# chenruduan/OAReactDiff

Measured on AMD Instinct MI355X. Metric: denoising_steps_per_sec, higher is better.
Workload: dtype f32; 1 GPU; EGNNDynamics.forward (LEFTNet H=196 R=96 L=6), B=64 reactions/GPU x 3 objects x 23 atoms, complete graph per reaction (N=4416, E=300288), T=1000 sampler step shape; batch_per_gpu=64, atoms_per_object=23, parallelism=replica x1 (no collective), launch=eager

## Files before the change

### oareactdiff_amd/_capi.py

```python
from __future__ import annotations

import ctypes as C
import os

from .build import LIB

OARD_MAX_OBJECTS = 8
ABI_VERSION = 2040
OARD_OK, OARD_EINVAL, OARD_ENOTCOMPLETE, OARD_EHIP, OARD_ENOMEM = 0, -1, -2, -3, -4
ERRORS = {OARD_EINVAL: "invalid argument / unsupported configuration", OARD_ENOTCOMPLETE: "topology is not complete-per-sample",
          OARD_EHIP: "HIP runtime error", OARD_ENOMEM: "workspace too small"}

PREC_GCL_BF16X3, PREC_EQUI_BF16X3, PREC_TRAIN_BF16X3 = 1, 2, 4
TAP_S, TAP_VEC, TAP_EDGE, TAP_POS_FRAME, TAP_DPOS, TAP_HOUT, TAP_LABELS, TAP_NE1 = 1, 2, 3, 4, 5, 6, 7, 8

EXPORTS = ["oard_version", "oard_supported", "oard_param_count", "oard_packed_bytes", "oard_pack_weights",
           "oard_topology_create", "oard_topology_destroy", "oard_topology_num_nodes", "oard_topology_num_edges",
           "oard_topology_num_inner_edges", "oard_topology_num_samples", "oard_topology_check_edge_index",
           "oard_workspace_bytes", "oard_forward", "oard_active_inner_edges", "oard_debug_lin3u_table", "oard_sampler_step", "oard_sampler_step_dev", "oard_tap", "oard_debug_stop_after", "oard_debug_option", "oard_timing_enable", "oard_timing_reset",
           "oard_timing_get",
           "oard_topology_create_parts", "oard_topology_export", "oard_tape_bytes", "oard_tape_entry", "oard_forward_train",
           "oard_packed_bwd_bytes", "oard_pack_weights_bwd", "oard_gcl_backward_dx", "oard_edge_node_sums",
           "oard_equi_backward_dx", "oard_scalarize_backward", "oard_equi_msg_backward", "oard_lin3u_forward", "oard_lin3u_backward", "oard_wgrad_scratch_bytes", "oard_wgrad",
           "oard_train_scratch_bytes", "oard_train_scratch_poison", "oard_train_scratch_entry", "oard_train_tail_backward",
# ... 46 lines not shown
        raise OardError(f"{LIB} not found: build it with `python -m oareactdiff_amd.build` "
                        "(there is no CPU fallback for the HIP backend)")
    L = C.CDLL(LIB)
    vp, i32, i64, sz = C.c_void_p, C.c_int32, C.c_int64, C.c_size_t
    cfgp = C.POINTER(OardConfig)
    L.oard_version.restype = C.c_int
    got = L.oard_version()
    if got != ABI_VERSION:
        raise OardError(f"{LIB} has ABI version {got}, this package expects {ABI_VERSION}: rebuild it "
                        "(`python -m oareactdiff_amd.build --force`, or the script that made the OARD_LIB build)")
    L.oard_supported.argtypes = [cfgp]; L.oard_supported.restype = C.c_int
    L.oard_param_count.argtypes = [cfgp]; L.oard_param_count.restype = sz
    L.oard_packed_bytes.argtypes = [cfgp]; L.oard_packed_bytes.restype = sz
    L.oard_pack_weights.argtypes = [cfgp, C.POINTER(vp), sz, vp, sz, vp]; L.oard_pack_weights.restype = C.c_int
    L.oard_topology_create.argtypes = [cfgp, C.POINTER(i64), C.POINTER(i64), i64, C.POINTER(vp)]
    L.oard_topology_create.restype = C.c_int
    L.oard_topology_destroy.argtypes = [vp]; L.oard_topology_destroy.restype = None
    for f in ("oard_topology_num_nodes", "oard_topology_num_edges", "oard_topology_num_inner_edges",
              "oard_topology_num_samples"):
        getattr(L, f).argtypes = [vp]; getattr(L, f).restype = i64
    L.oard_topology_check_edge_index.argtypes = [vp, vp, i64, vp, vp]; L.oard_topology_check_edge_index.restype = C.c_int
    L.oard_workspace_bytes.argtypes = [cfgp, vp]; L.oard_workspace_bytes.restype = sz
    L.oard_forward.argtypes = [cfgp, vp, vp, C.POINTER(vp), vp, C.c_int, vp, C.POINTER(vp), vp, sz, vp, vp]
    L.oard_forward.restype = C.c_int
    L.oard_debug_lin3u_table.argtypes = [cfgp, vp, C.c_int, vp, vp]; L.oard_debug_lin3u_table.restype = C.c_int
    L.oard_active_inner_edges.argtypes = [cfgp, vp, vp, sz, C.POINTER(i64), vp]; L.oard_active_inner_edges.restype = C.c_int
    L.oard_sampler_step.argtypes = [cfgp, vp, C.c_int, C.POINTER(vp), C.POINTER(vp), C.POINTER(vp), C.POINTER(vp),
                                    C.c_float, C.c_float, C.c_float, C.c_int, C.POINTER(vp), vp]
    L.oard_sampler_step.restype = C.c_int
    L.oard_sampler_step_dev.argtypes = [cfgp, vp, C.c_int, C.POINTER(vp), C.POINTER(vp), C.POINTER(vp), C.POINTER(vp), vp, C.c_int,
                                        C.POINTER(vp), vp]
    L.oard_sampler_step_dev.restype = C.c_int
    L.oard_tap.argtypes = [cfgp, vp, vp, C.c_int, C.c_int, vp, vp]; L.oard_tap.restype = C.c_int
    ci = C.c_int
    L.oard_topology_create_parts.argtypes = [cfgp, C.POINTER(i64), C.POINTER(i64), i64, ci, C.POINTER(vp)]
    L.oard_topology_create_parts.restype = ci
    L.oard_topology_export.argtypes = [vp, ci, vp, i64, vp]; L.oard_topology_export.restype = ci
    L.oard_tape_bytes.argtypes = [cfgp, vp]; L.oard_tape_bytes.restype = sz
    L.oard_tape_entry.argtypes = [cfgp, vp, ci, ci, C.POINTER(sz), C.POINTER(i64), C.POINTER(i64)]; L.oard_tape_entry.restype = ci
    L.oard_forward_train.argtypes = [cfgp, vp, vp, C.POINTER(vp), vp, ci, vp, C.POINTER(vp), vp, sz, vp, sz, vp, vp]
    L.oard_forward_train.restype = ci
    L.oard_packed_bwd_bytes.argtypes = [cfgp]; L.oard_packed_bwd_bytes.restype = sz
    L.oard_pack_weights_bwd.argtypes = [cfgp, C.POINTER(vp), sz, vp, sz, vp]; L.oard_pack_weights_bwd.restype = ci
    L.oard_gcl_backward_dx.argtypes = [cfgp, vp, vp, ci, vp, vp, vp, vp, vp, vp, vp, vp, vp]; L.oard_gcl_backward_dx.restype = ci
    L.oard_edge_node_sums.argtypes = [cfgp, vp, vp, vp, vp, vp]; L.oard_edge_node_sums.restype = ci
    L.oard_equi_backward_dx.argtypes = [cfgp, vp, vp, ci, vp, vp, vp, vp, vp]; L.oard_equi_backward_dx.restype = ci
    L.oard_scalarize_backward.argtypes = [cfgp, vp, vp, vp, vp, ci, vp, vp, vp, vp]; L.oard_scalarize_backward.restype = ci
    L.oard_equi_msg_backward.argtypes = [cfgp, vp, vp, ci, vp, vp, vp, vp, vp, vp, vp, vp, vp]; L.oard_equi_msg_backward.restype = ci
    L.oard_lin3u_forward.argtypes = [cfgp, vp, ci, vp, i64, vp, vp]; L.oard_lin3u_forward.restype = ci
    L.oard_lin3u_backward.argtypes = [cfgp, vp, ci, vp, vp, i64, vp, vp, vp, vp, vp, vp, vp]; L.oard_lin3u_backward.restype = ci
    L.oard_wgrad_scratch_bytes.argtypes = [ci, ci, i64]; L.oard_wgrad_scratch_bytes.restype = sz
    L.oard_wgrad.argtypes = [vp, ci, ci, ci, ci, ci, vp, ci, ci, ci, ci, ci, ci, i64, vp, vp, vp, sz, vp]; L.oard_wgrad.restype = ci
    pvp = C.POINTER(vp)
    L.oard_train_scratch_bytes.argtypes = [cfgp, vp]; L.oard_train_scratch_bytes.restype = sz
    L.oard_train_scratch_poison.argtypes = [cfgp, vp, vp, sz, vp]; L.oard_train_scratch_poison.restype = ci
    L.oard_train_scratch_entry.argtypes = [cfgp, vp, ci, C.POINTER(sz), C.POINTER(i64), C.POINTER(i64)]; L.oard_train_scratch_entry.restype = ci
    L.oard_train_tail_backward.argtypes = [cfgp, vp, vp, vp, vp, pvp, vp, vp, pvp, pvp, vp, sz, vp]; L.oard_train_tail_backward.restype = ci
    L.oard_train_layer_backward.argtypes = [cfgp, vp, vp, vp, vp, ci, vp, vp, vp, pvp, pvp, vp, sz, vp]; L.oard_train_layer_backward.restype = ci
    L.oard_train_init_backward.argtypes = [cfgp, vp, vp, vp, vp, pvp, vp, vp, pvp, pvp, vp, sz, vp]; L.oard_train_init_backward.restype = ci
    L.oard_train_stage_backward.argtypes = [cfgp, vp, vp, vp, vp, ci, ci, vp, vp, vp, vp, vp, vp, pvp, pvp, vp, sz, vp]
    L.oard_train_stage_backward.restype = ci
    L.oard_nan_replace.argtypes = [cfgp, vp, vp, pvp, pvp, vp]; L.oard_nan_replace.restype = ci
    pf, cf = C.POINTER(C.c_float), C.c_float
    L.oard_loss_prepare.argtypes = [cfgp, vp, pvp, pvp, pvp, pvp, vp, vp, ci, pf, pf, ci, ci, pvp, pvp, vp]; L.oard_loss_prepare.restype = ci
    L.oard_loss_terms.argtypes = [cfgp, vp, pvp, pvp, pvp, pvp, pvp, vp, vp, ci, pf, pf, pf, ci, ci, vp, vp, pvp, vp]; L.oard_loss_terms.restype = ci
    cd = C.c_double
    L.oard_adamw_step.argtypes = [vp, vp, vp, vp, vp, i64, cd, cd, cd, cd, cd, i64, ci, cd, vp]; L.oard_adamw_step.restype = ci
    L.oard_adamw_step_dev.argtypes = [vp, vp, vp, vp, vp, i64, cd, cd, cd, cd, cd, ci, ci, vp, ci, vp, vp, vp, vp]; L.oard_adamw_step_dev.restype = ci
    L.oard_library_stream.argtypes = [ci, pvp]; L.oard_library_stream.restype = ci
    L.oard_graph_create.argtypes = [cfgp, vp, vp, i64, vp, i64, pvp]; L.oard_graph_create.restype = ci
    L.oard_graph_destroy.argtypes = [vp]; L.oard_graph_destroy.restype = None
    L.oard_graph_num_nodes.argtypes = [vp]; L.oard_graph_num_nodes.restype = i64
    L.oard_graph_num_edges.argtypes = [vp]; L.oard_graph_num_edges.restype = i64
    L.oard_graph_object_rows.argtypes = [vp, ci]; L.oard_graph_object_rows.restype = i64
    L.oard_graph_is_complete.argtypes = [vp]; L.oard_graph_is_complete.restype = ci
    L.oard_graph_workspace_bytes.argtypes = [cfgp, vp]; L.oard_graph_workspace_bytes.restype = sz
    L.oard_graph_forward.argtypes = [cfgp, vp, pvp, sz, pvp, vp, ci, vp, pvp, vp, sz, vp, vp]; L.oard_graph_forward.restype = ci
    L.oard_debug_stop_after.argtypes = [C.c_int]; L.oard_debug_stop_after.restype = C.c_int
    L.oard_debug_option.argtypes = [C.c_char_p, C.c_int]; L.oard_debug_option.restype = C.c_int
    L.oard_timing_enable.argtypes = [C.c_int]; L.oard_timing_enable.restype = C.c_int
    L.oard_timing_reset.argtypes = []; L.oard_timing_reset.restype = C.c_int
    L.oard_timing_get.argtypes = [C.c_char_p, C.POINTER(C.c_double), C.POINTER(i64)]; L.oard_timing_get.restype = C.c_int
    for env, opt in (("OARD_GCL_VARIANT", b"gcl_variant"), ("OARD_EQUI_VARIANT", b"equi_variant"),
                     ("OARD_NODE_VARIANT", b"node_variant"), ("OARD_GCL_SKIP", b"gcl_skip"), ("OARD_EQUI_SKIP", b"equi_skip"), ("OARD_EQUI_L0_SKIP", b"equi_l0_skip"), ("OARD_GCL_PERSIST", b"gcl_persist"), ("OARD_GCL_GRID", b"gcl_grid"), ("OARD_PARTS", b"parts"), ("OARD_SEQUENTIAL", b"sequential"), ("OARD_POISON", b"poison"), ("OARD_AUTO_SMALL", b"auto_small"), ("OARD_AUTO_TINY", b"auto_tiny"), ("OARD_NPB", b"npb"),
                     ("OARD_WGRAD_WGS", b"wgrad_wgs"), ("OARD_WGRAD_LDS", b"wgrad_lds"), ("OARD_WGRAD_T16", b"wgrad_t16"), ("OARD_WGRAD_QUEUE", b"wgrad_queue"), ("OARD_GATE_FOLD", b"gate_fold"), ("OARD_WGRAD_SHAPES", b"wgrad_shapes"), ("OARD_TRAIN_DUAL", b"train_dual"), ("OARD_SMALL_SPLIT", b"small_split"),
                     ("OARD_SKIP_FAMILIES", b"skip_families")):
        if os.environ.get(env) not in (None, ""):
            check(L.oard_debug_option(opt, int(os.environ[env])), f"oard_debug_option({opt.decode()})")
    _lib = L
    return L


def timing_get(family: str):
    ms, n = C.c_double(0.0), C.c_int64(0)
    check(lib().oard_timing_get(family.encode(), C.byref(ms), C.byref(n)), "oard_timing_get")
    return ms.value, n.value
```

### oareactdiff_amd/csrc/oard_edge_p.h

```cpp
#pragma once
#include "oard_edge_v1.h"

template <class D, bool DO_S1, bool DO_S3, bool TRAIN = false>
__global__ __launch_bounds__(512, 2) void k_gcl_edge_p(TopoDev tp, const float* __restrict__ stream,
                                                       const float* __restrict__ P, const float* __restrict__ Q,
                                                       const float* __restrict__ u0, const float* __restrict__ c0,
                                                       long long r0, long long r1, const float* ew_in, float* ew_out,
                                                       float* __restrict__ mbuf, GclTape tape) {
    extern __shared__ __attribute__((aligned(16))) float smem[];
    constexpr int WAVES = 8, GP = 2, RING = 3, DIST = RING - 1;
    using S = GclStream<D, GP>;
    constexpr int HT = D::HT, WB = D::WB, G1 = S::G1, G2 = S::G2;
    constexpr bool TAIL1 = S::TAIL1, ROWS4 = S::ROWS4;
    constexpr int P0 = DO_S1 ? 0 : S::NP1, PEND = DO_S3 ? S::NPH : S::NP1 + S::NP2, NPR = PEND - P0;
    static_assert(NPR >= DIST, "a round must be at least as long as the prefetch distance");
    static_assert(HT >= 2, "the phase barrier sits inside the first chain of a phase");
    constexpr int BAR_AT = OARD_BAR_AT < HT / 2 ? OARD_BAR_AT : HT / 2;

    const int lane = threadIdx.x & 63, g = lane >> 4;
    const int wave = __builtin_amdgcn_readfirstlane(threadIdx.x >> 6);

    const long long WT = (r1 - r0 + 15) >> 4, NH = (WT + 3) >> 2;
    const long long hb0 = NH * blockIdx.x / gridDim.x, hb1 = NH * (blockIdx.x + 1) / gridDim.x;
    const int nh = (int)(hb1 - hb0), nr = (nh + 1) >> 1;
    if (nr == 0) return;
    auto is_half = [&](int r) -> bool { return 2 * r + 1 == nh; };
    auto active_in = [&](int r) -> bool { return !(is_half(r) && wave < 4); };
    auto row_of = [&](int r) -> size_t {
        const int slot = is_half(r) ? wave - 4 : wave;
        const long long c = r0 + (((hb0 + 2 * r) << 2) + slot) * 16 + (lane & 15);
        return (size_t)((slot >= 0 && c < r1) ? c : tp.E);
    };

    SlabPrefetch<WAVES, S::SLAB, 1, 1, RING> pf;
    pf.wave = wave;
    pf.lane_off = (unsigned)lane * 16u;
    int gp = 0;
    const float* strm = stream;
    const float* c0r = c0;
    const float* u0r = u0;
    auto pf_local = [&](int q, int at, bool ok) {
        int start = 0, n = 0;
        if (ok) {
            if (q < S::NP1) { start = q * GP * G1; n = min(GP, WB - q * GP) * G1; }
            else if (q < S::NP1 + S::NP2) { const int k = q - S::NP1; start = S::C1 + k * GP * G2; n = min(GP, S::NG2 - k * GP) * G2; }
            else { const int k = q - S::NP1 - S::NP2; start = S::C1 + S::C2 + k * GP * G2; n = min(GP, WB - k * GP) * G2; }
        }
        pf.begin(strm, smem, at, start, n);
    };
    bool more = nr > 1;
    auto pf_ahead = [&](int lp) {
        int q = lp + DIST;
        bool ok = true;
        if (q >= PEND) { q -= NPR; ok = more; }
        pf_local(q, gp + DIST, ok);
    };
    auto slab_of = [&](int p) -> int { return p % RING; };
    auto A = [&](int j) -> f4 { return *reinterpret_cast<const f4*>(smem + ((size_t)slab_of(gp) * S::SLAB + j) * 256 + lane * 4); };
    auto SL = [&]() -> const float* { return smem + (size_t)slab_of(gp) * S::SLAB * 256 + lane * 4; };

    pf_local(P0, 0, true);
    pf.flush();
    pf_local(P0 + 1 < PEND ? P0 + 1 : P0, 1, P0 + 1 < PEND || more);
    pf.flush();

    size_t e = 0;
    const float* erow = nullptr;
    float* orow = nullptr;
    f4 h1[HT];
    f4 xn[GP];
    auto set_rows = [&](size_t row) {
        e = row;
        erow = ew_in + e * D::WP + 4 * g;
        orow = ew_out + e * D::WP + 4 * g;
    };
    auto load_xn = [&](f4 (&x)[GP], const float* er) {
#pragma unroll
        for (int gg = 0; gg < GP; ++gg) x[gg] = (DO_S1 && gg < WB) ? ld_edge(er + 16 * gg) : f4zero();
    };
    size_t eid = 0;
    int src = 0, tgt = 0;
    auto load_h1 = [&]() {
#pragma unroll
        for (int t = 0; t < HT; ++t) {
            if (DO_S1) h1[t] = f4zero();
            else h1[t] = ld_blk(P, src, D::HP, t, lane) + ld_blk(Q, tgt, D::HP, t, lane) + ld_vec(u0r, t, lane);
        }
    };
    if (active_in(0)) {
        set_rows(row_of(0));
        eid = (size_t)tp.row_eid[e]; src = tp.row_src[e]; tgt = tp.row_tgt[e];
        load_h1();
        load_xn(xn, erow);
    }
    PHASE_BARRIER();

    int bar_left = 0;
    for (int r = 0; r < nr; ++r) {
        more = r + 1 < nr;
        strm = stream; c0r = c0; u0r = u0;
        asm volatile("" : "+s"(strm), "+s"(c0r), "+s"(u0r));
        if (!active_in(r)) {
            for (int lp = P0; lp < PEND; ++lp) { PHASE_BARRIER(); pf_ahead(lp); pf.flush(); ++gp; }
            continue;
        }
        const bool nxt = more && active_in(r + 1);
        int src_n = 0, tgt_n = 0;
        size_t eid_n = 0;
        f4 xn_n[GP];
        f4 hp[HT], hq[HT];
        int lp = P0;

        f4 h1x = f4zero();
        f4 xm[GP];
        auto s1_phase = [&](int p1, const f4 (&x)[GP], f4 (&xnext)[GP], auto last_tag) {
            constexpr bool LAST = decltype(last_tag)::value;
            auto post = [&]() {
                pf_ahead(lp);
                if (p1 + 1 < S::NP1) {
#pragma unroll
                    for (int gg = 0; gg < GP; ++gg) {
                        const int b = (p1 + 1) * GP + gg;
                        if (b < WB) xnext[gg] = ld_edge(erow + 16 * b);
                    }
                }
                if (LAST) {
                    pf.flush();
#pragma unroll
                    for (int t = 0; t < HT; ++t) { hp[t] = ld_blk(P, src, D::HP, t, lane); hq[t] = ld_blk(Q, tgt, D::HP, t, lane); }
                }
            };
            auto hook = [&]() { if (bar_left > 0 && --bar_left == 0) { PHASE_BARRIER(); post(); } pf.tick(); };
            bar_left = BAR_AT;
#pragma unroll
            for (int gg = 0; gg < GP; ++gg)
                if (p1 * GP + gg < WB) chain_kouter<HT, ROWS4>(SL(), gg * G1, x[gg], h1, h1x, hook);
            if (bar_left > 0) { bar_left = 0; PHASE_BARRIER(); post(); }
            pf.flush();
            ++gp; ++lp;
        };
        if (DO_S1) {
            int p1 = 0;
            for (; p1 + 2 < S::NP1; p1 += 2) { s1_phase(p1, xn, xm, std::false_type{}); s1_phase(p1 + 1, xm, xn, std::false_type{}); }
            if (p1 + 2 == S::NP1) { s1_phase(p1, xn, xm, std::false_type{}); s1_phase(p1 + 1, xm, xn, std::true_type{}); }
            else s1_phase(p1, xn, xm, std::true_type{});
        }
        if (ROWS4 && DO_S1) {
            const f4 v = reduce_g(h1[HT - 1] + h1x);
            h1[HT - 1] = g == 0 ? v : f4zero();
        }
        if (DO_S1) {
#pragma unroll
            for (int t = 0; t < HT; ++t) h1[t] += hp[t] + hq[t];
        }
        if (TRAIN) {
#pragma unroll
            for (int t = 0; t < HT; ++t) st_blk(tape.z1, e, D::HP, t, lane, h1[t]);
        }
#pragma unroll
        for (int t = 0; t < HT; ++t) h1[t] = silu4(h1[t]);
        const float h1_tail = TAIL1 ? tail_compact(h1[HT - 1], lane) : 0.f;

        f4 m[HT];
        f4 on[GP];
        f4 pz2[TRAIN ? GP : 1];
        float m_tail = 0.f;
#pragma unroll
        for (int p2 = 0; p2 < S::NP2; ++p2) {
            auto post = [&]() {
                if (TRAIN && p2 > 0) {
#pragma unroll
                    for (int gg = 0; gg < GP; ++gg)
                        if ((p2 - 1) * GP + gg < HT) st_blk(tape.z2, e, D::HP, (p2 - 1) * GP + gg, lane, pz2[gg]);
                }
                pf_ahead(lp);
                if (DO_S3 && p2 == S::NP2 - 1) {
#pragma unroll
                    for (int gg = 0; gg < GP; ++gg)
                        on[gg] = gg < WB ? (DO_S1 ? ld_edge(erow + 16 * gg) : ld_f4(c0r + 16 * gg + 4 * g)) : f4zero();
                }
            };
            auto hook = [&]() { if (bar_left > 0 && --bar_left == 0) { PHASE_BARRIER(); post(); } pf.tick(); };
            bar_left = BAR_AT;
#pragma unroll
            for (int gg = 0; gg < GP; ++gg) {
                const int tg = p2 * GP + gg;
                if (tg < S::NG2) {
                    const f4 bias = A(gg * G2);
                    f4 acc;
                    if (ROWS4 && tg >= HT - 1) {
                        acc = reduce_g(tg < HT ? chain_tile4<HT>(SL(), gg * G2 + 1, h1, bias, hook)
                                               : chain_tile4<HT>(SL(), gg * G2 + 1, m, bias, hook));
                        if (tg < HT && g != 0) acc = f4zero();
                    } else {
                        acc = tg < HT ? chain_tile<HT, TAIL1>(SL(), gg * G2 + 1, h1, bias, h1_tail, hook)
                                      : chain_tile<HT, TAIL1>(SL(), gg * G2 + 1, m, bias, m_tail, hook);
                    }
                    if (tg < HT) {
                        if (TRAIN) pz2[gg] = acc;
                        m[tg] = silu4(acc);
                        if (TAIL1 && tg == HT - 1) m_tail = tail_compact(m[HT - 1], lane);
                    } else {
                        const float a = ROWS4 ? acc.x : __shfl(acc.x, lane & 15, 64);
                        if (TRAIN && g == 0) tape.att[e] = a;
                        const float gate = silu1(a);
#pragma unroll
                        for (int t = 0; t < HT; ++t) m[t] *= gate;
                        m_tail *= gate;
                    }
                }
            }
            if (bar_left > 0) { bar_left = 0; PHASE_BARRIER(); post(); }
            pf.flush();
            ++gp; ++lp;
        }

        if (TRAIN) {
#pragma unroll
            for (int gg = 0; gg < GP; ++gg)
                if ((S::NP2 - 1) * GP + gg < HT) st_blk(tape.z2, e, D::HP, (S::NP2 - 1) * GP + gg, lane, pz2[gg]);
        }
        if (!DO_S3) {
#pragma unroll
            for (int t = 0; t < HT; ++t) st_blk(mbuf, eid, D::HP, t, lane, m[t]);
        } else {
            f4 pend[GP], pendz[TRAIN ? GP : 1];
            f4 om[GP];
            auto s3_phase = [&](int p3, const f4 (&o)[GP], f4 (&onext)[GP], auto last_tag) {
                constexpr bool LAST = decltype(last_tag)::value;
                auto post = [&]() {
                    if (p3 == 0) {
#pragma unroll
                        for (int t = 0; t < HT; ++t) st_blk(mbuf, eid, D::HP, t, lane, m[t]);
                    } else {
#pragma unroll
                        for (int gg = 0; gg < GP; ++gg) {
                            st_f4(orow + 16 * ((p3 - 1) * GP + gg), pend[gg]);
                            if (TRAIN) st_f4(tape.z3 + e * D::WP + 4 * g + 16 * ((p3 - 1) * GP + gg), pendz[gg]);
                        }
                    }
                    pf_ahead(lp);
                    if (p3 + 1 < S::NP3) {
#pragma unroll
                        for (int gg = 0; gg < GP; ++gg) {
                            const int t = (p3 + 1) * GP + gg;
                            if (t < WB) onext[gg] = DO_S1 ? ld_edge(erow + 16 * t) : ld_f4(c0r + 16 * t + 4 * g);
                        }
                    }
                    if (nxt) {
                        if (p3 == 0) {
                            const size_t en = row_of(r + 1);
                            src_n = tp.row_src[en]; tgt_n = tp.row_tgt[en]; eid_n = (size_t)tp.row_eid[en];
                        }
                        if (LAST) load_xn(xn_n, ew_in + row_of(r + 1) * D::WP + 4 * g);
                    }
                };
                auto hook = [&]() { if (bar_left > 0 && --bar_left == 0) { PHASE_BARRIER(); post(); } pf.tick(); };
                bar_left = BAR_AT;
#pragma unroll
                for (int gg = 0; gg < GP; ++gg) {
                    const int t = p3 * GP + gg;
                    if (t < WB) {
                        const f4 z = chain_tile<HT, TAIL1>(SL(), gg * G2 + 1, m, A(gg * G2), m_tail, hook);
                        if (TRAIN) pendz[gg] = z;
                        pend[gg] = o[gg] + silu4(z);
                    }
                }
                if (bar_left > 0) { bar_left = 0; PHASE_BARRIER(); post(); }
                pf.flush();
                ++gp; ++lp;
            };
            {
                int p3 = 0;
                for (; p3 + 2 < S::NP3; p3 += 2) { s3_phase(p3, on, om, std::false_type{}); s3_phase(p3 + 1, om, on, std::false_type{}); }
                if (p3 + 2 == S::NP3) { s3_phase(p3, on, om, std::false_type{}); s3_phase(p3 + 1, om, on, std::true_type{}); }
                else s3_phase(p3, on, om, std::true_type{});
            }
#pragma unroll
            for (int gg = 0; gg < GP; ++gg) {
                const int t = (S::NP3 - 1) * GP + gg;
                if (t < WB) {
                    st_f4(orow + 16 * t, pend[gg]);
                    if (TRAIN) st_f4(tape.z3 + e * D::WP + 4 * g + 16 * t, pendz[gg]);
                }
            }
        }

        if (nxt) {
            set_rows(row_of(r + 1));
            if (DO_S3) {
                eid = eid_n; src = src_n; tgt = tgt_n;
#pragma unroll
                for (int gg = 0; gg < GP; ++gg) xn[gg] = xn_n[gg];
            } else {
                eid = (size_t)tp.row_eid[e]; src = tp.row_src[e]; tgt = tp.row_tgt[e];
                load_xn(xn, erow);
            }
            load_h1();
        }
    }
}
```

### oareactdiff_amd/csrc/oard_edge_v1.h

```cpp
#pragma once
#include "oard_kernels.h"

typedef __attribute__((address_space(3))) void* lds_ptr_t;
typedef const __attribute__((address_space(1))) void* gbl_ptr_t;

OARD_DEV void glds16(const float* gsrc_lane, float* lds_chunk);
OARD_DEV void glds16u(const float* chunk_uniform, unsigned lane_byte_off, float* lds_chunk) {
    glds16(reinterpret_cast<const float*>(reinterpret_cast<const char*>(chunk_uniform) + lane_byte_off), lds_chunk);
}
OARD_DEV void glds16(const float* gsrc_lane, float* lds_chunk) {
#ifndef OARD_ABL_NODMA_INSTR
    __builtin_amdgcn_global_load_lds((gbl_ptr_t)gsrc_lane, (lds_ptr_t)lds_chunk, 16, 0, 0);
#else
    asm volatile("" :: "v"(gsrc_lane), "s"(lds_chunk));
#endif
}

OARD_DEV void phase_barrier() {
    asm volatile("s_waitcnt vmcnt(0)" ::: "memory");
#ifndef OARD_ABL_NOBARRIER
    __syncthreads();
#endif
}

#ifdef OARD_PHASE_PROBE
OARD_DEVVAR __device__ unsigned long long g_phase_probe[8];
#define PROBE_DECL long long pr_t0_ = clock64(), pr_wait_ = 0, pr_bar_ = 0, pr_n_ = 0;
#define PHASE_BARRIER() do { const long long a_ = clock64(); asm volatile("s_waitcnt vmcnt(0)" ::: "memory"); const long long b_ = clock64(); \
        __syncthreads(); const long long c_ = clock64(); pr_wait_ += b_ - a_; pr_bar_ += c_ - b_; ++pr_n_; } while (0)
#define PROBE_END(pf) do { if ((threadIdx.x & 63) == 0) { atomicAdd(&g_phase_probe[0], 1ull); atomicAdd(&g_phase_probe[1], (unsigned long long)(clock64() - pr_t0_)); \
        atomicAdd(&g_phase_probe[2], (unsigned long long)pr_wait_); atomicAdd(&g_phase_probe[3], (unsigned long long)pr_bar_); \
        atomicAdd(&g_phase_probe[4], (unsigned long long)(pf).dma_cyc); atomicAdd(&g_phase_probe[5], (unsigned long long)(pf).dma_n); \
        atomicAdd(&g_phase_probe[6], (unsigned long long)pr_n_); if ((threadIdx.x >> 6) < (blockDim.x >> 7)) atomicAdd(&g_phase_probe[7], (unsigned long long)pr_bar_); } } while (0)
#else
#define PROBE_DECL
#define PHASE_BARRIER() phase_barrier()
#define PROBE_END(pf) do {} while (0)
#endif

#ifdef OARD_TIMELINE
#define TL_MAX 1024
OARD_DEVVAR __device__ long long g_timeline[16][TL_MAX];
#define TL_DECL const bool tl_on_ = DO_S1 && DO_S3 && blockIdx.x == gridDim.x / 2 && (threadIdx.x & 63) == 0; int tl_n_ = 0;
#define TL(code) do { if (tl_on_ && tl_n_ < TL_MAX) g_timeline[threadIdx.x >> 6][tl_n_++] = (clock64() << 3) | (code); } while (0)
#define TL_END() do { if (tl_on_ && tl_n_ < TL_MAX) g_timeline[threadIdx.x >> 6][tl_n_] = 0; } while (0)
#else
#define TL_DECL
#define TL(code) do {} while (0)
#define TL_END() do {} while (0)
#endif

OARD_DEV void mma_pair(f4 a0, f4 b0, f4& c0, f4 a1, f4 b1, f4& c1) {
    c0 = __builtin_amdgcn_mfma_f32_16x16x4f32(a0.x, b0.x, c0, 0, 0, 0);
    c1 = __builtin_amdgcn_mfma_f32_16x16x4f32(a1.x, b1.x, c1, 0, 0, 0);
    c0 = __builtin_amdgcn_mfma_f32_16x16x4f32(a0.y, b0.y, c0, 0, 0, 0);
    c1 = __builtin_amdgcn_mfma_f32_16x16x4f32(a1.y, b1.y, c1, 0, 0, 0);
    c0 = __builtin_amdgcn_mfma_f32_16x16x4f32(a0.z, b0.z, c0, 0, 0, 0);
    c1 = __builtin_amdgcn_mfma_f32_16x16x4f32(a1.z, b1.z, c1, 0, 0, 0);
    c0 = __builtin_amdgcn_mfma_f32_16x16x4f32(a0.w, b0.w, c0, 0, 0, 0);
    c1 = __builtin_amdgcn_mfma_f32_16x16x4f32(a1.w, b1.w, c1, 0, 0, 0);
}

OARD_DEV void mma4_chunk(f4 a, f4 b, f4& c0, f4& c1) {
    c0 = __builtin_amdgcn_mfma_f32_4x4x1f32(a.x, b.x, c0, 0, 0, 0);
    c1 = __builtin_amdgcn_mfma_f32_4x4x1f32(a.y, b.y, c1, 0, 0, 0);
    c0 = __builtin_amdgcn_mfma_f32_4x4x1f32(a.z, b.z, c0, 0, 0, 0);
    c1 = __builtin_amdgcn_mfma_f32_4x4x1f32(a.w, b.w, c1, 0, 0, 0);
}
OARD_DEV f4 reduce_g(f4 v) {
    f4 r;
#pragma unroll
    for (int c = 0; c < 4; ++c) {
        float x = v[c];
        x += __shfl_xor(x, 16, 64);
        x += __shfl_xor(x, 32, 64);
        r[c] = x;
    }
    return r;
}

OARD_DEV f4 lds_a(const float* sl, int j) { return *reinterpret_cast<const f4*>(sl + j * 256); }

struct NoHook { OARD_DEV void operator()() const {} };
template <int KB, bool TAIL, class Hook>
OARD_DEV f4 chain_tile(const float* sl, int j0, const f4 (&in)[KB], f4 init, float tail, Hook hook) {
    static_assert(!TAIL || (KB & 1), "compact tail needs an odd number of chunks");
    f4 c0 = init, c1 = f4zero();
// ... 32 lines not shown
        a0 = n0; a1 = n1;
        __builtin_amdgcn_sched_barrier(0);
    }
    if (KB & 1) mma4_chunk(a0, in[KB - 1], c0, c1);
    return c0 + c1;
}
template <int MT, bool ROWS4, class Hook>
OARD_DEV void chain_kouter(const float* sl, int j0, f4 x, f4 (&acc)[MT], f4& extra, Hook hook) {
    static_assert(!ROWS4 || (MT & 1), "the 4-row tile must be the odd one");
    f4 a0 = lds_a(sl, j0), a1 = MT > 1 ? lds_a(sl, j0 + 1) : f4zero();
#pragma unroll
    for (int t = 0; t + 1 < MT; t += 2) {
        f4 n0 = a0, n1 = a1;
        if (t + 2 < MT) n0 = lds_a(sl, j0 + t + 2);
        if (t + 3 < MT) n1 = lds_a(sl, j0 + t + 3);
        mma_pair(a0, x, acc[t], a1, x, acc[t + 1]);
        hook();
        a0 = n0; a1 = n1;
    }
    if (MT & 1) {
        if (ROWS4) mma4_chunk(a0, x, acc[MT - 1], extra);
        else acc[MT - 1] = mma_chunk(a0, x, acc[MT - 1]);
    }
}
template <int MT, class Hook = NoHook>
OARD_DEV void chain_kouter(const float* sl, int j0, f4 x, f4 (&acc)[MT], Hook hook = Hook()) {
    f4 unused = f4zero();
    chain_kouter<MT, false, Hook>(sl, j0, x, acc, unused, hook);
}

#ifndef OARD_PF_HALF
#define OARD_PF_HALF 1
#endif
#ifndef OARD_PF_PERIOD
#define OARD_PF_PERIOD 1
#endif
template <int WAVES, int SLAB, int HALF = OARD_PF_HALF, int PERIOD = OARD_PF_PERIOD, int RING = 2>
struct SlabPrefetch {
    static constexpr int IW = (HALF && WAVES >= 8) ? WAVES / 2 : WAVES;
    static constexpr int KMAX = (SLAB + IW - 1) / IW;
    const float* src;
    float* dst;
    unsigned lane_off;
    int n, k, next, wave;
#ifdef OARD_PHASE_PROBE
    long long dma_cyc = 0, dma_n = 0;
#endif
    OARD_DEV void begin(const float* stream, float* smem, int phase, int first_chunk, int n_chunks) {
        src = stream + (size_t)first_chunk * 256;
        dst = smem + (size_t)(RING == 2 ? (phase & 1) : (phase % RING)) * SLAB * 256;
        n = wave < IW ? n_chunks : 0; k = 0; next = 1 + ((IW == WAVES && wave >= WAVES / 2) ? 1 : 0);
    }
    OARD_DEV void one() {
#ifdef OARD_ABL_NOHOOK
        k = KMAX;
        return;
#endif
        const int j = wave + k * IW;
#ifdef OARD_PHASE_PROBE
        if (j < n) { const long long a_ = clock64(); glds16u(src + (size_t)j * 256, lane_off, dst + j * 256); dma_cyc += clock64() - a_; ++dma_n; }
#else
        if (j < n) glds16u(src + (size_t)j * 256, lane_off, dst + j * 256);
#endif
        ++k;
    }
#ifdef OARD_ABL_BURST
    OARD_DEV void tick() {}
#else
#ifdef OARD_ABL_NOHOOK
    OARD_DEV void tick() {}
#else
    OARD_DEV void tick() { if (--next == 0) { one(); next = PERIOD; } }
#endif
#endif
    OARD_DEV void flush() { while (k < KMAX) one(); }
};

#ifdef OARD_ABL_NOEDGELOAD
OARD_DEV f4 ld_edge(const float* p) { return (f4){0.25f, -0.5f, 0.125f, 1.0f}; }
#else
OARD_DEV f4 ld_edge(const float* p) { return ld_f4(p); }
#endif

template <class D, int GP>
struct GclStream {
    static constexpr int HT = D::HT, WB = D::WB, G1 = HT, G2 = HT + 1, NG2 = HT + 1;
    static constexpr bool TAIL1 = (D::H % 16) >= 1 && (D::H % 16) <= 4 && HT >= 3 && (HT & 1);
    static constexpr bool ROWS4 = TAIL1;
    static constexpr int SLAB = GP * G2;
    static constexpr int NP1 = (WB + GP - 1) / GP, NP2 = (NG2 + GP - 1) / GP, NP3 = NP1, NPH = NP1 + NP2 + NP3;
    static constexpr int C1 = WB * G1, C2 = NG2 * G2, C3 = WB * G2, CHUNKS = C1 + C2 + C3;
    static constexpr size_t LDS_BYTES = (size_t)2 * SLAB * 1024;
};

struct GclTape {
    float* z1;
    float* z2;
    float* att;
    float* z3;
};

OARD_DEV float tail_compact(f4 v, int lane) {
    const int e = lane & 15, g = lane >> 4;
    const float t0 = __shfl(v.x, e, 64), t1 = __shfl(v.y, e, 64), t2 = __shfl(v.z, e, 64), t3 = __shfl(v.w, e, 64);
    return g == 0 ? t0 : (g == 1 ? t1 : (g == 2 ? t2 : t3));
}
#ifndef OARD_BAR_AT
#define OARD_BAR_AT 2
#endif
template <class D, int WAVES, int GP, bool DO_S1, bool DO_S3, bool TRAIN, int MINW = 2, int RING = 2>
__global__ __launch_bounds__(WAVES * 64, MINW) void k_gcl_edge_v1(TopoDev tp, const float* __restrict__ stream,
                                                               const float* __restrict__ P, const float* __restrict__ Q,
                                                               const float* __restrict__ u0, const float* __restrict__ c0,
                                                               long long r0, long long r1, const float* ew_in, float* ew_out,
                                                               float* __restrict__ mbuf, GclTape tape) {
    extern __shared__ __attribute__((aligned(16))) float smem[];
    using S = GclStream<D, GP>;
    constexpr int HT = D::HT, WB = D::WB, G1 = S::G1, G2 = S::G2;
    constexpr bool TAIL1 = S::TAIL1, ROWS4 = S::ROWS4;
    const int lane = threadIdx.x & 63, g = lane >> 4;
    const int wave = __builtin_amdgcn_readfirstlane(threadIdx.x >> 6);
    PROBE_DECL
    TL_DECL
    TL(0);
    static_assert(RING == 2 || RING == 3, "two slabs (barrier at the phase start) or three (barrier inside the phase)");
    static_assert(RING == 2 || HT >= 2, "the phase barrier must sit inside the FIRST chain of a phase (S3 stores the previous phase's results behind it)");
    constexpr int DIST = RING - 1;
    constexpr int BAR_AT = OARD_BAR_AT < HT / 2 ? OARD_BAR_AT : HT / 2;
    SlabPrefetch<WAVES, S::SLAB, OARD_PF_HALF, OARD_PF_PERIOD, RING> pf;
    pf.wave = wave;
    pf.lane_off = (unsigned)lane * 16u;
    auto pf_begin = [&](int p) {
        int start = 0, n = 0;
        if (p < S::NP1) { start = p * GP * G1; n = min(GP, WB - p * GP) * G1; }
        else if (p < S::NP1 + S::NP2) { const int q = p - S::NP1; start = S::C1 + q * GP * G2; n = min(GP, S::NG2 - q * GP) * G2; }
        else if (p < S::NPH && DO_S3) { const int q = p - S::NP1 - S::NP2; start = S::C1 + S::C2 + q * GP * G2; n = min(GP, WB - q * GP) * G2; }
        pf.begin(stream, smem, p, start, n);
#ifdef OARD_ABL_BURST
        pf.flush();
#endif
    };
    int bar_left = 0;
    auto slab_of = [&](int p) -> int { return RING == 2 ? (p & 1) : (p % RING); };
    auto A = [&](int p, int j) -> f4 {
        return *reinterpret_cast<const f4*>(smem + ((size_t)slab_of(p) * S::SLAB + j) * 256 + lane * 4);
    };
    auto SL = [&](int p) -> const float* { return smem + (size_t)slab_of(p) * S::SLAB * 256 + lane * 4; };

    const long long c = r0 + ((long long)blockIdx.x * WAVES + wave) * 16 + (lane & 15);
    const size_t e = (size_t)(c < r1 ? c : tp.E);
    const float* erow = ew_in + e * D::WP + 4 * g;
    float* orow = ew_out + e * D::WP + 4 * g;
    f4 h1[HT];
    const size_t eid = (size_t)tp.row_eid[e];
    {
        const int src = tp.row_src[e], tgt = tp.row_tgt[e];
#pragma unroll
        for (int t = 0; t < HT; ++t) {
            h1[t] = ld_blk(P, src, D::HP, t, lane) + ld_blk(Q, tgt, D::HP, t, lane);
            if (!DO_S1) h1[t] += ld_vec(u0, t, lane);
        }
    }
    f4 xn[GP];
#pragma unroll
    for (int gg = 0; gg < GP; ++gg) xn[gg] = (DO_S1 && gg < WB) ? ld_edge(erow + 16 * gg) : f4zero();
    int p = DO_S1 ? 0 : S::NP1;
    pf_begin(p);
    pf.flush();
    if (RING == 3) { pf_begin(p + 1); pf.flush(); PHASE_BARRIER(); }

    f4 h1x = f4zero();
    f4 xm[GP];
    auto s1_phase = [&](int p1, const f4 (&x)[GP], f4 (&xnext)[GP]) {
        auto post = [&]() {
            TL(1);
            pf_begin(p + DIST);
            if (p1 + 1 < S::NP1) {
#pragma unroll
                for (int gg = 0; gg < GP; ++gg) {
                    const int b = (p1 + 1) * GP + gg;
                    if (b < WB) xnext[gg] = ld_edge(erow + 16 * b);
                }
            }
        };
        auto hook = [&]() { if (RING == 3 && bar_left > 0 && --bar_left == 0) { PHASE_BARRIER(); post(); } pf.tick(); };
        if (RING == 2) { PHASE_BARRIER(); post(); } else bar_left = BAR_AT;
#pragma unroll
        for (int gg = 0; gg < GP; ++gg)
            if (p1 * GP + gg < WB) { TL(2); chain_kouter<HT, ROWS4>(SL(p), gg * G1, x[gg], h1, h1x, hook); TL(3); }
        TL(4);
        if (RING == 3 && bar_left > 0) { bar_left = 0; PHASE_BARRIER(); post(); }
        pf.flush();
        ++p;
    };
    if (DO_S1) {
        int p1 = 0;
        for (; p1 + 1 < S::NP1; p1 += 2) { s1_phase(p1, xn, xm); s1_phase(p1 + 1, xm, xn); }
        if (p1 < S::NP1) s1_phase(p1, xn, xm);
    }
    if (ROWS4 && DO_S1) {
        const f4 v = reduce_g(h1[HT - 1] + h1x);
        h1[HT - 1] = g == 0 ? v : f4zero();
    }
    if (TRAIN) {
#pragma unroll
        for (int t = 0; t < HT; ++t) st_blk(tape.z1, e, D::HP, t, lane, h1[t]);
    }
#pragma unroll
    for (int t = 0; t < HT; ++t) h1[t] = silu4(h1[t]);
    const float h1_tail = TAIL1 ? tail_compact(h1[HT - 1], lane) : 0.f;

    f4 m[HT];
    f4 on[GP];
    f4 pz2[TRAIN ? GP : 1];
    float m_tail = 0.f;
#pragma unroll
    for (int p2 = 0; p2 < S::NP2; ++p2, ++p) {
        auto post = [&]() {
            TL(1);
            if (TRAIN && p2 > 0) {
#pragma unroll
                for (int gg = 0; gg < GP; ++gg)
                    if ((p2 - 1) * GP + gg < HT) st_blk(tape.z2, e, D::HP, (p2 - 1) * GP + gg, lane, pz2[gg]);
            }
            pf_begin(p + DIST);
            if (DO_S3 && p2 == S::NP2 - 1) {
#pragma unroll
                for (int gg = 0; gg < GP; ++gg)
                    on[gg] = gg < WB ? (DO_S1 ? ld_edge(erow + 16 * gg) : ld_f4(c0 + 16 * gg + 4 * g)) : f4zero();
            }
        };
        auto hook = [&]() { if (RING == 3 && bar_left > 0 && --bar_left == 0) { PHASE_BARRIER(); post(); } pf.tick(); };
        if (RING == 2) { PHASE_BARRIER(); post(); } else bar_left = BAR_AT;
#pragma unroll
        for (int gg = 0; gg < GP; ++gg) {
            const int tg = p2 * GP + gg;
            if (tg < S::NG2) {
                const f4 bias = A(p, gg * G2);
                TL(2);
                f4 acc;
                if (ROWS4 && tg >= HT - 1) {
                    acc = reduce_g(tg < HT ? chain_tile4<HT>(SL(p), gg * G2 + 1, h1, bias, hook)
                                           : chain_tile4<HT>(SL(p), gg * G2 + 1, m, bias, hook));
                    if (tg < HT && g != 0) acc = f4zero();
                } else {
                    acc = tg < HT ? chain_tile<HT, TAIL1>(SL(p), gg * G2 + 1, h1, bias, h1_tail, hook)
                                  : chain_tile<HT, TAIL1>(SL(p), gg * G2 + 1, m, bias, m_tail, hook);
                }
                TL(3);
                if (tg < HT) {
                    if (TRAIN) pz2[gg] = acc;
                    m[tg] = silu4(acc);
                    if (TAIL1 && tg == HT - 1) m_tail = tail_compact(m[HT - 1], lane);
                } else {
                    const float a = ROWS4 ? acc.x : __shfl(acc.x, lane & 15, 64);
                    if (TRAIN && g == 0) tape.att[e] = a;
                    const float gate = silu1(a);
#pragma unroll
                    for (int t = 0; t < HT; ++t) m[t] *= gate;
                    m_tail *= gate;
                }
            }
        }
        TL(4);
        if (RING == 3 && bar_left > 0) { bar_left = 0; PHASE_BARRIER(); post(); }
        pf.flush();
    }
    if (TRAIN) {
#pragma unroll
        for (int gg = 0; gg < GP; ++gg)
            if ((S::NP2 - 1) * GP + gg < HT) st_blk(tape.z2, e, D::HP, (S::NP2 - 1) * GP + gg, lane, pz2[gg]);
    }
    if (!DO_S3) {
#pragma unroll
        for (int t = 0; t < HT; ++t) st_blk(mbuf, eid, D::HP, t, lane, m[t]);
        PROBE_END(pf);
        TL_END();
        return;
    }
    f4 pend[GP], pendz[TRAIN ? GP : 1];
    f4 om[GP];
    auto s3_phase = [&](int p3, const f4 (&o)[GP], f4 (&onext)[GP]) {
        auto post = [&]() {
            TL(1);
            if (p3 == 0) {
#pragma unroll
                for (int t = 0; t < HT; ++t) st_blk(mbuf, eid, D::HP, t, lane, m[t]);
            } else {
#pragma unroll
                for (int gg = 0; gg < GP; ++gg) {
                    st_f4(orow + 16 * ((p3 - 1) * GP + gg), pend[gg]);
                    if (TRAIN) st_f4(tape.z3 + e * D::WP + 4 * g + 16 * ((p3 - 1) * GP + gg), pendz[gg]);
                }
            }
            pf_begin(p + DIST);
            if (p3 + 1 < S::NP3) {
#pragma unroll
                for (int gg = 0; gg < GP; ++gg) {
                    const int t = (p3 + 1) * GP + gg;
                    if (t < WB)
                        onext[gg] = DO_S1 ? ld_edge(erow + 16 * t) : ld_f4(c0 + 16 * t + 4 * g);
                }
            }
        };
        auto hook = [&]() { if (RING == 3 && bar_left > 0 && --bar_left == 0) { PHASE_BARRIER(); post(); } pf.tick(); };
        if (RING == 2) { PHASE_BARRIER(); post(); } else bar_left = BAR_AT;
#pragma unroll
        for (int gg = 0; gg < GP; ++gg) {
            const int t = p3 * GP + gg;
            if (t < WB) {
                TL(2);
                const f4 z = chain_tile<HT, TAIL1>(SL(p), gg * G2 + 1, m, A(p, gg * G2), m_tail, hook);
                TL(3);
                if (TRAIN) pendz[gg] = z;
                pend[gg] = o[gg] + silu4(z);
            }
        }
        TL(4);
        if (RING == 3 && bar_left > 0) { bar_left = 0; PHASE_BARRIER(); post(); }
        pf.flush();
        ++p;
    };
    {
        int p3 = 0;
        for (; p3 + 1 < S::NP3; p3 += 2) { s3_phase(p3, on, om); s3_phase(p3 + 1, om, on); }
        if (p3 < S::NP3) s3_phase(p3, on, om);
    }
#pragma unroll
    for (int gg = 0; gg < GP; ++gg) {
        const int t = (S::NP3 - 1) * GP + gg;
        if (t < WB) {
            st_f4(orow + 16 * t, pend[gg]);
            if (TRAIN) st_f4(tape.z3 + e * D::WP + 4 * g + 16 * t, pendz[gg]);
        }
    }
    PROBE_END(pf);
    TL_END();
}

template <class D>
struct EquiStream {
    static constexpr int WB = D::WB, D1T = D::D1T, RB = D::RB, HT = D::HT;
    static constexpr int G1 = D1T, G2 = 1 + D1T + RB, NG2 = 3 * HT;
    static constexpr bool ROWS4 = (D::H % 16) >= 1 && (D::H % 16) <= 4;
    static constexpr int SLAB = G2 > G1 ? G2 : G1;
    static constexpr int NPH = WB + NG2;
    static constexpr int C1 = WB * G1, CHUNKS = C1 + NG2 * G2;
    static constexpr size_t LDS_BYTES = (size_t)2 * SLAB * 1024;
};

template <class D, int WAVES, bool TRAIN>
__global__ __launch_bounds__(WAVES * 64) void k_equi_edge_v1(TopoDev tp, const float* __restrict__ stream,
                                                             const float* __restrict__ dp0b,
                                                             const float* __restrict__ ew, const float* __restrict__ rbuf,
                                                             float* __restrict__ qbuf, float* __restrict__ zd1,
                                                             float* __restrict__ cdbuf, ActList al, int skip_mid) {
    extern __shared__ __attribute__((aligned(16))) float smem[];
    using S = EquiStream<D>;
    constexpr int WB = D::WB, D1T = D::D1T, RB = D::RB, HT = D::HT, G1 = S::G1, G2 = S::G2;
    const int lane = threadIdx.x & 63, g = lane >> 4;
    const int wave = __builtin_amdgcn_readfirstlane(threadIdx.x >> 6);

    SlabPrefetch<WAVES, S::SLAB, 0, 3> pf;
    pf.wave = wave;
    pf.lane_off = (unsigned)lane * 16u;
    const bool skip = !TRAIN && skip_mid != 0;
    auto pf_begin = [&](int ph) {
        pf.begin(stream, smem, ph, ph * G1, G1);
    };
    auto pf_begin_t2 = [&](int ph, int slot) {
        pf.begin(stream, smem, ph, S::C1 + slot * G2, slot < S::NG2 ? G2 : 0);
    };
    auto next_slot = [&](int i) -> int { return i + ((skip && i % 3 == 0) ? 2 : 1); };
    auto hook = [&]() { pf.tick(); };
    auto A = [&](int p, int j) -> f4 {
        return *reinterpret_cast<const f4*>(smem + ((size_t)(p & 1) * S::SLAB + j) * 256 + lane * 4);
    };
    auto SL = [&](int p) -> const float* { return smem + (size_t)(p & 1) * S::SLAB * 256 + lane * 4; };

    const long long n_cols = al.n != nullptr ? (long long)*al.n : tp.A;
    if ((long long)blockIdx.x * WAVES * 16 >= n_cols) return;
    const long long c = ((long long)blockIdx.x * WAVES + wave) * 16 + (lane & 15);
    const bool live = c < n_cols;
    const size_t a = (size_t)(live ? (al.rows != nullptr ? (long long)al.rows[c] : c) : tp.A);
    const float* erow = ew + (live ? a : (size_t)tp.E) * D::WP + 4 * g;
    f4 d1[D1T];
#pragma unroll
    for (int t = 0; t < D1T; ++t) d1[t] = ld_vec(dp0b, t, lane);
    f4 rb[RB];
#pragma unroll
    for (int b = 0; b < RB; ++b) rb[b] = ld_blk(rbuf, a, D::RP, b, lane);
    f4 xn = ld_f4(erow);
    pf_begin(0);
    pf.flush();

    int p = 0;
    for (int b = 0; b < WB; ++b, ++p) {
        phase_barrier();
        const f4 x = xn;
        if (b + 1 < WB) pf_begin(p + 1); else pf_begin_t2(p + 1, 0);
        if (b + 1 < WB) xn = ld_f4(erow + 16 * (b + 1));
        chain_kouter<D1T>(SL(p), 0, x, d1, hook);
// ... 125 lines not shown
```

### oareactdiff_amd/csrc/oard_hip.hip

```cpp
#include <algorithm>
#include <cmath>
#include <cstdio>
#include <cstring>
#include <map>
#include <string>
#include <vector>
#include <mutex>
#include <chrono>
#include <utility>

#include "oard_kernels.h"
#include "oard_edge_v1.h"
#include "oard_edge_p.h"
#include "oard_wgrad_t16.h"
#include "oard_edge_b3.h"
#ifdef OARD_EXPERIMENTS
#include "oard_edge_fp.h"
#endif
#include "oard_node_v1.h"
#include "oard_edge_small.h"
#include "oard_edge_bwd.h"
#include "oard_node_bwd.h"
#include "oard_rows.h"
#include "oard_inst.h"

#define OARD_VERSION 2040
#ifdef OARD_EXPERIMENTS
static constexpr bool kV0 = true;
#else
static constexpr bool kV0 = false;
#endif

#define HIP_TRY(x) do { hipError_t e_ = (x); if (e_ != hipSuccess) { \
    fprintf(stderr, "liboard_hip: %s failed: %s (%s:%d)\n", #x, hipGetErrorString(e_), __FILE__, __LINE__); \
    return OARD_EHIP; } } while (0)

namespace {
enum Family { F_GCL_EDGE = 0, F_EQUI_EDGE, F_NODE, F_INIT, F_OTHER, F_GCL_BWD, F_EQUI_BWD, F_WGRAD, F_COUNT };
const char* kFamilyNames[F_COUNT] = {"gcl_edge", "equi_edge", "node", "init", "other", "gcl_edge_bwd", "equi_edge_bwd", "wgrad"};
struct TimingRec { hipEvent_t a, b; int fam; };
struct Timing {
    bool on = false;
    std::vector<TimingRec> recs;
    std::vector<hipEvent_t> pool;
    double total_ms[F_COUNT] = {0};
    long long launches[F_COUNT] = {0};
    hipEvent_t get() {
        if (!pool.empty()) { hipEvent_t e = pool.back(); pool.pop_back(); return e; }
        hipEvent_t e; (void)hipEventCreate(&e); return e;
    }
    void flush() {
        for (auto& r : recs) {
            (void)hipEventSynchronize(r.b);
            float ms = 0.f;
            (void)hipEventElapsedTime(&ms, r.a, r.b);
            total_ms[r.fam] += ms; launches[r.fam] += 1;
            pool.push_back(r.a); pool.push_back(r.b);
        }
        recs.clear();
    }
} g_timing;
int g_stop_after = 0;
int g_gcl_variant = 2;
int g_equi_variant = 2;
int g_sequential = 0;
int g_auto_tiny = 8;
int g_auto_small = 4;
int g_npb = 0;
int g_poison = 0;
int g_equi_l0_skip = 1;
int g_equi_l0_taken = 0;
int g_parts = 0;
int g_small_split = 128;
int g_wgrad_shapes = 3;
int g_wgrad_t16 = 256;
int g_wgrad_lds = 256;
int g_wgrad_wgs = 512;
int g_gcl_persist = 1;
int g_gcl_grid = 0;
int g_equi_skip = 1;
int g_gcl_skip = 1;
int g_node_variant = 1;
int g_skip_families = 0;

struct ScopedLaunch {
    hipStream_t st; hipEvent_t a; int fam; bool on;
    ScopedLaunch(int f, hipStream_t s) : st(s), fam(f), on(g_timing.on) {
        if (on) { a = g_timing.get(); (void)hipEventRecord(a, st); }
    }
    ~ScopedLaunch() {
        if (on) { hipEvent_t b = g_timing.get(); (void)hipEventRecord(b, st); g_timing.recs.push_back({a, b, fam}); }
    }
};
#define LAUNCH(fam, kern, grid, block, stream, ...) do { ScopedLaunch sl_(fam, stream); if (!((g_skip_families >> (fam)) & 1)) \
    hipLaunchKernelGGL(kern, dim3((unsigned)(grid)), dim3(block), 0, stream, __VA_ARGS__); } while (0)
#define LAUNCH2(fam, kern, gx, gy, block, stream, ...) do { ScopedLaunch sl_(fam, stream); if (!((g_skip_families >> (fam)) & 1)) \
    hipLaunchKernelGGL(kern, dim3((unsigned)(gx), (unsigned)(gy)), dim3(block), 0, stream, __VA_ARGS__); } while (0)

#ifndef OARD_DIMS_LIST
#define OARD_DIMS_LIST X(196, 96) X(32, 8) X(32, 32)
#endif

inline size_t align_up(size_t x, size_t a) { return (x + a - 1) / a * a; }
inline long long cdiv(long long a, long long b) { return (a + b - 1) / b; }

bool config_ok(const oard_config* c) {
    if (!c) return false;
    bool dims = false;
#define X(h, r) dims = dims || (c->hidden == (h) && c->num_radial == (r));
    OARD_DIMS_LIST
#undef X
    if (!dims) return false;
    if (c->num_layers < 1 || c->num_layers > OARD_MAX_LAYERS) return false;
    if (c->in_hidden < 1 || c->in_hidden > 16) return false;
    if (c->n_obj < 1 || c->n_obj > OARD_MAX_OBJECTS) return false;
    if (c->pos_dim != 3 || (c->reflect_equiv != 0 && c->reflect_equiv != 1)) return false;
    if (c->precision & ~(OARD_PREC_GCL_BF16X3 | OARD_PREC_EQUI_BF16X3 | OARD_PREC_TRAIN_BF16X3)) return false;
    const int emb = c->in_hidden - (c->condition_time ? 1 : 0) - (c->condition_nf > 0 ? c->condition_nf : 0);
    if (emb < 1) return false;
    for (int k = 0; k < c->n_obj; ++k) {
        const int d = c->node_nf[k] - 3;
        if (d < 1 || d > 16) return false;
        const int a = c->enc_alias[k];
        if (a < 0 || a >= c->n_obj || c->node_nf[a] != c->node_nf[k]) return false;
    }
    return true;
}
int embed_dim(const oard_config* c) {
    return c->in_hidden - (c->condition_time ? 1 : 0) - (c->condition_nf > 0 ? c->condition_nf : 0);
}

PackOff make_layout(const oard_config* c) {
    const RDims d(c->hidden, c->num_radial);
    PackOff po;
    memset(&po, 0, sizeof(po));
    size_t cur = 0;
    auto take = [&](size_t n) { size_t o = cur; cur = align_up(cur + n, 64); return o; };
    auto mat = [&](int MT, int KB) { return take((size_t)MT * KB * 256); };
    const int emb = embed_dim(c);
    po.emb = mat(d.HT, 1); po.emb_b = take(d.HP);
    po.nbemb = mat(d.HT, 1); po.nbemb_b = take(d.HP);
    po.s2v = mat(d.HT, d.HT); po.s2v_b = take(d.HP);
    po.rl0 = mat(d.HT, d.RB); po.rl0_b = take(d.HP);
    po.rl2 = mat(d.HT, d.HT); po.rl2_b = take(d.HP);
    po.lin3 = take((size_t)d.H4 * 5 + 1);
    po.pe0 = take((size_t)d.H2 * 3);
    po.pe1 = mat(d.HT, d.PB);
    po.embout = mat(1, d.HT); po.embout_b = take(16);
    po.v1p = mat(d.HT, d.HT); po.v2p = take(d.HP);
    po.un0 = mat(d.HT, 2 * d.HT); po.un0_b = take(d.HP);
    po.un2 = mat(1, d.HT); po.un2_b = take(16);
    po.c0row = take(d.WP);
    po.u0 = take(d.HP);
// ... 68 lines not shown
        j.block0 = blocks;
        blocks += cdiv((long long)std::max<size_t>(work, 1), 256);
        jobs.push_back(j);
    }
    void matrix(int src, int src_ld, int col_off, int msl, int msp, int ms, int ksl, int ksp, int ks, int MT, int KB,
                size_t dst, size_t tstride = 0, size_t bstride = 256, int perm_ht = 0, int transpose = 0, int tail_compact = 0,
                int rows4 = 0) {
        if (tstride == 0) tstride = (size_t)KB * 256;
        GenJob j;
        memset(&j, 0, sizeof(j));
        j.type = 0;
        j.m = PackJob{p[src], src_ld, col_off, msl, msp, ms, ksl, ksp, ks, MT, KB, dst, tstride, bstride, perm_ht, transpose, rows4, tail_compact};
        push(j, (size_t)MT * KB * 256);
    }
    void nat(int src, int src_ld, int col_off, int M, int K, int MT, int KB, size_t dst) {
        matrix(src, src_ld, col_off, M, MT * 16, 1, K, KB * 16, 1, MT, KB, dst);
    }
    void vec(int src, int sect_len, int sect_pad, int sects, int n_dst, size_t dst) {
        GenJob j;
        memset(&j, 0, sizeof(j));
        j.type = 1; j.src = src >= 0 ? p[src] : nullptr; j.dst = dst; j.sect_len = sect_len; j.sect_pad = sect_pad; j.sects = sects; j.n = n_dst;
        push(j, (size_t)n_dst);
    }
    void bias_chunks(int src, int sect_len, int sect_pad, int sects, int n_tiles, size_t dst, size_t tstride,
                     int perm_ht = 0) {
        GenJob j;
        memset(&j, 0, sizeof(j));
        j.type = 2; j.src = p[src]; j.dst = dst; j.sect_len = sect_len; j.sect_pad = sect_pad; j.sects = sects; j.n = n_tiles * 256;
        j.tstride = tstride; j.perm_ht = perm_ht;
        push(j, (size_t)n_tiles * 256);
    }
    void raw(int src, int n, size_t dst) {
        GenJob j;
        memset(&j, 0, sizeof(j));
        j.type = 3; j.src = p[src]; j.dst = dst; j.n = n;
        push(j, (size_t)n);
    }
    int flush() {
        if (jobs.empty()) return OARD_OK;
        struct Cached { std::vector<GenJob> host; GenJob* dev = nullptr; size_t cap = 0; };
        static std::mutex mu;
        static std::map<std::pair<const void*, int>, Cached> cache;
        int devid = 0;
        (void)hipGetDevice(&devid);
        const GenJob* table = nullptr;
        {
            std::lock_guard<std::mutex> lk(mu);
            Cached& c = cache[{(const void*)blob, devid}];
            const bool same = c.host.size() == jobs.size() && memcmp(c.host.data(), jobs.data(), jobs.size() * sizeof(GenJob)) == 0;
            if (!same) {
                HIP_TRY(hipStreamSynchronize(st));
                if (c.cap < jobs.size()) {
                    if (c.dev) (void)hipFree(c.dev);
                    HIP_TRY(hipMalloc((void**)&c.dev, jobs.size() * sizeof(GenJob)));
                    c.cap = jobs.size();
                }
                HIP_TRY(hipMemcpy(c.dev, jobs.data(), jobs.size() * sizeof(GenJob), hipMemcpyHostToDevice));
                c.host = jobs;
            }
            table = c.dev;
        }
        hipLaunchKernelGGL(k_pack_all, dim3((unsigned)blocks), dim3(256), 0, st, table, (int)jobs.size(), blob);
        jobs.clear();
        blocks = 0;
        return OARD_OK;
    }
};
#define OARD_SMALL_MAX_EDGES (512 * 16 * 16)
struct SmallScratch { float* a; float* b; };
static thread_local SmallScratch t_small = {nullptr, nullptr};
static WsOff make_ws(const oard_config* c, const TopoDev& td) {
    const RDims d(c->hidden, c->num_radial);
    const size_t N = td.N, E = td.E + 1, A = td.A + 1;
    WsOff w;
    size_t cur = 0;
    auto take = [&](size_t bytes) { size_t o = cur; cur = align_up(cur + bytes, 256); return o; };
    w.pos = take(N * 3 * 4); w.pf64 = take(N * 3 * 8); w.pf32 = take(N * 3 * 4); w.x1 = take(N * 3 * 4);
    w.pp0 = take(N * 4); w.labels = take(N * 4); w.hin = take(N * 16 * 4);
    w.zemb = take(N * d.HP * 4); w.nb = take(N * d.HP * 4); w.s = take(N * d.HP * 4); w.s1 = take(N * d.HP * 4);
    w.ne1 = take(N * 3 * d.HP * 4); w.xh = take(N * d.HP * 4); w.P = take(N * d.HP * 4); w.Q = take(N * d.HP * 4);
    w.xq = take(N * 3 * d.HP * 4); w.vec = take(N * 3 * d.HP * 4); w.vec2 = take(N * 3 * d.HP * 4); w.v2buf = take(N * 3 * d.HP * 4);
    w.sc0 = take(N * d.HP * 4); w.vdot = take(N * d.HP * 4);
    w.geo = take(A * GEO_STRIDE * 4); w.d64 = take(A * 8); w.rbuf = take(A * d.RP * 4);
    w.ew = take(E * d.WP * 4); w.mbuf = take(E * d.HP * 4);
    w.xmsg = take(A * d.HP * 4); w.vmsg = take(A * 3 * d.HP * 4);
    w.dpos = take(N * 3 * 4); w.hout = take(N * 16 * 4);
    w.al_rows = take(A * 4); w.al_src = take(A * 4); w.al_pre = take(A * 4); w.al_cnt = take((size_t)cdiv((long long)td.A, 256) * 4 + 4); w.al_n = take(4);
    w.d1s = take((size_t)cdiv((long long)td.A, 128) * 8 * d.D1T * 1024);
    w.small_a = w.small_b = 0;
    if (E <= (size_t)OARD_SMALL_MAX_EDGES) {
        w.small_a = take(A * d.D1P * 4);
    }
    w.total = cur;
    return w;
}



template <class K>
int set_lds(K kernel, size_t bytes) {
    HIP_TRY(hipFuncSetAttribute((const void*)kernel, hipFuncAttributeMaxDynamicSharedMemorySize, (int)bytes));
    return OARD_OK;
}

#define LAUNCH_LDS(fam, kern, grid, block, lds, stream, ...) do { \
    static bool attr_done_[64] = {}; \
    int dev_ = 0; (void)hipGetDevice(&dev_); dev_ &= 63; \
    if (!attr_done_[dev_]) { int rc_ = set_lds(kern, lds); if (rc_ != OARD_OK) return rc_; attr_done_[dev_] = true; } \
    ScopedLaunch sl_(fam, stream); if (!((g_skip_families >> (fam)) & 1)) \
    hipLaunchKernelGGL(kern, dim3((unsigned)(grid)), dim3(block), lds, stream, __VA_ARGS__); } while (0)

#define GCL_CASE(id, WV_, GP_) case id: { \
        LAUNCH_LDS(F_GCL_EDGE, (k_gcl_edge_v1<D, WV_, GP_, S1, S3, false>), cdiv(r1 - r0, 16 * WV_), WV_ * 64, \
                   (GclStream<D, GP_>::LDS_BYTES), st, tp, stream, P, Q, u0, c0, r0, r1, ew_in, ew_out, mbuf, GclTape{}); return OARD_OK; }
#define GCL_RING3(TRAIN_, tape_) do { \
        LAUNCH_LDS(F_GCL_EDGE, (k_gcl_edge_v1<D, 8, 2, S1, S3, TRAIN_, 2, 3>), cdiv(r1 - r0, 16 * 8), 8 * 64, \
                   (GclStream<D, 2>::LDS_BYTES / 2 * 3), st, tp, stream, P, Q, u0, c0, r0, r1, ew_in, ew_out, mbuf, tape_); return OARD_OK; } while (0)
static int device_cus() {
    static int cus[64] = {};
    int d = 0;
    (void)hipGetDevice(&d);
    d &= 63;
    if (!cus[d]) {
        int n = 0;
        if (hipDeviceGetAttribute(&n, hipDeviceAttributeMultiprocessorCount, d) != hipSuccess || n < 1) { (void)hipGetLastError(); n = 256; }
        cus[d] = n;
    }
    return cus[d];
}
template <class D, bool S1, bool S3>
int launch_gcl_v1s(int prec, int variant, int conc, const TopoDev& tp, const float* wb, const LayerOff& lo, const float* stream, const float* P, const float* Q, const float* u0,
                   const float* c0, long long r0, long long r1, const float* ew_in, float* ew_out, float* mbuf, const GclTape* tape, hipStream_t st) {
    if (r1 <= r0) return OARD_OK;
    if (tape && (prec & OARD_PREC_TRAIN_BF16X3)) {
        LAUNCH_LDS(F_GCL_EDGE, (k_gcl_edge_b3<D, S1, S3, true>), cdiv(r1 - r0, 16 * 8), 8 * 64, (GclB3Stream<D>::LDS_BYTES), st, tp,
                   wb + lo.gcl_b3, P, Q, u0, c0, r0, r1, ew_in, ew_out, mbuf, *tape);
        return OARD_OK;
    }
    if (tape) {
#ifdef OARD_EXPERIMENTS
        if (variant == 7) {
            LAUNCH_LDS(F_GCL_EDGE, (k_gcl_edge_v1<D, 8, 2, S1, S3, true>), cdiv(r1 - r0, 16 * 8), 8 * 64,
                       (GclStream<D, 2>::LDS_BYTES), st, tp, stream, P, Q, u0, c0, r0, r1, ew_in, ew_out, mbuf, *tape);
            return OARD_OK;
        }
#endif
        if (g_gcl_persist) {
            const long long nhalf = cdiv(cdiv(r1 - r0, 16), 4);
            const long long want = g_gcl_grid > 0 ? g_gcl_grid : (g_gcl_grid < 0 ? cdiv(nhalf, 2LL * -g_gcl_grid) : device_cus());
            LAUNCH_LDS(F_GCL_EDGE, (k_gcl_edge_p<D, S1, S3, true>), std::min(nhalf, want), 8 * 64, (GclStream<D, 2>::LDS_BYTES / 2 * 3), st,
                       tp, stream, P, Q, u0, c0, r0, r1, ew_in, ew_out, mbuf, *tape);
            return OARD_OK;
        }
        GCL_RING3(true, *tape);
    }
    if (variant == 2 && cdiv(r1 - r0, 16) * conc <= 1024LL * g_auto_small) variant = 3;
    if ((variant == 2 || variant == 3) && cdiv(r1 - r0, 16) * conc <= 512LL * g_auto_tiny) variant = 6;
    if (variant == 6) {
        LAUNCH_LDS(F_GCL_EDGE, (k_gcl_edge_small<D, 8, S1, S3>), cdiv(r1 - r0, 16), 512, (GclSmall<D>::LDS_BYTES), st,
                   tp, wb, lo, P, Q, u0, c0, r0, r1, ew_out, mbuf);
        return OARD_OK;
    }
    switch (variant) {
        case 2:
            if (prec & OARD_PREC_GCL_BF16X3) {
                LAUNCH_LDS(F_GCL_EDGE, (k_gcl_edge_b3<D, S1, S3>), cdiv(r1 - r0, 16 * 8), 8 * 64, (GclB3Stream<D>::LDS_BYTES), st, tp,
                           wb + lo.gcl_b3, P, Q, u0, c0, r0, r1, ew_in, ew_out, mbuf, GclTape{});
                return OARD_OK;
            }
            if (g_gcl_persist > 1 || (g_gcl_persist == 1 && conc == 1)) {
                const long long nhalf = cdiv(cdiv(r1 - r0, 16), 4);
                const long long want = g_gcl_grid > 0 ? g_gcl_grid : (g_gcl_grid < 0 ? cdiv(nhalf, 2LL * -g_gcl_grid) : (conc > 1 ? std::max(1, device_cus() / 2) : device_cus()));
                LAUNCH_LDS(F_GCL_EDGE, (k_gcl_edge_p<D, S1, S3>), std::min(nhalf, want), 8 * 64, (GclStream<D, 2>::LDS_BYTES / 2 * 3), st,
                           tp, stream, P, Q, u0, c0, r0, r1, ew_in, ew_out, mbuf, GclTape{});
                return OARD_OK;
            }
            GCL_RING3(false, GclTape{});
        GCL_CASE(3, 4, 2)
#ifdef OARD_EXPERIMENTS
        GCL_CASE(7, 8, 2)
        case 4: {
            LAUNCH_LDS(F_GCL_EDGE, (k_gcl_edge_fp<D, 8, 2, S1, S3, false>), cdiv(r1 - r0, 16 * 8), 8 * 64,
                       (GclRing<D, 2, 4>::LDS_BYTES), st, tp, stream, P, Q, u0, c0, r0, r1, ew_in, ew_out, mbuf, GclTape{}); return OARD_OK; }
        case 5: {
            LAUNCH_LDS(F_GCL_EDGE, (k_gcl_edge_fp<D, 8, 2, S1, S3, false, 3>), cdiv(r1 - r0, 16 * 8), 8 * 64,
                       (GclRing<D, 2, 3>::LDS_BYTES), st, tp, stream, P, Q, u0, c0, r0, r1, ew_in, ew_out, mbuf, GclTape{}); return OARD_OK; }
        GCL_CASE(8, 8, 3)
        GCL_CASE(9, 8, 4)
        case 10: { LAUNCH_LDS(F_GCL_EDGE, (k_gcl_edge_v1<D, 12, 1, S1, S3, false, 3>), cdiv(r1 - r0, 16 * 12), 12 * 64,
                              (GclStream<D, 1>::LDS_BYTES), st, tp, stream, P, Q, u0, c0, r0, r1, ew_in, ew_out, mbuf, GclTape{}); return OARD_OK; }
        case 11: { LAUNCH_LDS(F_GCL_EDGE, (k_gcl_edge_v1<D, 12, 2, S1, S3, false, 3>), cdiv(r1 - r0, 16 * 12), 12 * 64,
                              (GclStream<D, 2>::LDS_BYTES), st, tp, stream, P, Q, u0, c0, r0, r1, ew_in, ew_out, mbuf, GclTape{}); return OARD_OK; }
        case 12: { LAUNCH_LDS(F_GCL_EDGE, (k_gcl_edge_v1<D, 4, 1, S1, S3, false, 3>), cdiv(r1 - r0, 16 * 4), 4 * 64,
                              (GclStream<D, 1>::LDS_BYTES), st, tp, stream, P, Q, u0, c0, r0, r1, ew_in, ew_out, mbuf, GclTape{}); return OARD_OK; }
#endif
        default: return OARD_EINVAL;
    }
}
template <class D>
int launch_gcl_v1(int prec, int variant, int conc, const TopoDev& tp, const float* wb, const LayerOff& lo, const float* stream, const float* P, const float* Q, const float* u0,
                  const float* c0, bool first, bool last, const float* ew_in, float* ew_out, float* mbuf, const GclTape* tape, hipStream_t st) {
    const long long A = tp.A, E = tp.E;
    int rc;
    const bool skip = g_gcl_skip || tape;
    if (!skip || (!first && !last)) return launch_gcl_v1s<D, true, true>(prec, variant, conc, tp, wb, lo, stream, P, Q, u0, c0, 0, E, ew_in, ew_out, mbuf, tape, st);
    rc = launch_gcl_v1s<D, true, true>(prec, variant, conc, tp, wb, lo, stream, P, Q, u0, c0, 0, A, ew_in, ew_out, mbuf, tape, st);
    if (rc != OARD_OK) return rc;
    if (first && last) return launch_gcl_v1s<D, false, false>(prec, variant, conc, tp, wb, lo, stream, P, Q, u0, c0, A, E, ew_in, ew_out, mbuf, tape, st);
    if (first) return launch_gcl_v1s<D, false, true>(prec, variant, conc, tp, wb, lo, stream, P, Q, u0, c0, A, E, ew_in, ew_out, mbuf, tape, st);
    return launch_gcl_v1s<D, true, false>(prec, variant, conc, tp, wb, lo, stream, P, Q, u0, c0, A, E, ew_in, ew_out, mbuf, tape, st);
}
static int equi_v1_shape(int prec, int variant, int conc, long long A, const float* d1s) {
    if (variant == 2 && cdiv(A, 16) * conc <= 512LL * g_auto_small) variant = 1;
    if ((variant == 2 || variant == 1) && cdiv(A, 16) * conc <= 512LL * g_auto_tiny) variant = 4;
    if (variant == 2 && (prec & OARD_PREC_EQUI_BF16X3) && d1s) variant = 5;
    return variant;
}
#define EQUI_CASE(id, WV_, SKIP_) case id: { \
        LAUNCH_LDS(F_EQUI_EDGE, (k_equi_edge_v1<D, WV_, false>), cdiv(tp.A, 16 * WV_), WV_ * 64, (EquiStream<D>::LDS_BYTES), st, \
                   tp, stream, dp0b, ew, rbuf, qbuf, nullptr, nullptr, al, SKIP_); return OARD_OK; }
template <class D>
int launch_equi_v1(int prec, int variant, int conc, const TopoDev& tp, const float* wb, const LayerOff& lo, const float* stream, const float* dp0b, const float* ew,
                   const float* rbuf, float* qbuf, float* zd1, float* cd, hipStream_t st, float* d1s = nullptr, ActList al = ActList{}, bool skip_mid = false) {
    if (zd1 && (prec & OARD_PREC_TRAIN_BF16X3) && d1s) {
        LAUNCH_LDS(F_EQUI_EDGE, (k_equi_edge_b3<D, true>), cdiv(tp.A, 16 * 8), 8 * 64, (EquiB3Stream<D>::LDS_BYTES), st, tp, wb + lo.equi_b3,
                   dp0b, wb + lo.dp2b, ew, rbuf, qbuf, d1s, zd1, cd, ActList{});
        return OARD_OK;
    }
    if (zd1) {
        LAUNCH_LDS(F_EQUI_EDGE, (k_equi_edge_v1<D, 8, true>), cdiv(tp.A, 16 * 8), 8 * 64, (EquiStream<D>::LDS_BYTES), st,
                   tp, stream, dp0b, ew, rbuf, qbuf, zd1, cd, ActList{}, 0);
        return OARD_OK;
    }
    variant = equi_v1_shape(prec, variant, conc, tp.A, d1s);
    if (skip_mid && variant != 2) return OARD_EINVAL;
    if (variant == 4) {
        if (t_small.a && cdiv(tp.A, 16) * conc <= g_small_split) {
            const long long tiles = cdiv(tp.A, 16);
            LAUNCH_LDS(F_EQUI_EDGE, (k_equi_small_s1<D, 8>), tiles * cdiv(D::D1T, 8), 512, (size_t)D::WB * 1024, st,
                       tp, wb, lo, ew, t_small.a);
            LAUNCH_LDS(F_EQUI_EDGE, (k_equi_small_s2<D, 8>), tiles * cdiv(3 * D::HT, 8), 512, (size_t)(D::D1T + D::RB) * 1024, st,
                       tp, wb, lo, (const float*)t_small.a, rbuf, qbuf);
            return OARD_OK;
        }
        LAUNCH_LDS(F_EQUI_EDGE, (k_equi_edge_small<D, 8>), cdiv(tp.A, 16), 512, (EquiSmall<D>::LDS_BYTES), st,
                   tp, wb, lo, ew, rbuf, qbuf);
        return OARD_OK;
    }
    if (variant == 5) {
        LAUNCH_LDS(F_EQUI_EDGE, (k_equi_edge_b3<D>), cdiv(tp.A, 16 * 8), 8 * 64, (EquiB3Stream<D>::LDS_BYTES), st, tp, wb + lo.equi_b3,
                   dp0b, wb + lo.dp2b, ew, rbuf, qbuf, d1s, nullptr, nullptr, al);
        return OARD_OK;
    }
    switch (variant) {
        EQUI_CASE(1, 4, 0)
        EQUI_CASE(2, 8, skip_mid ? 1 : 0)
        default: return OARD_EINVAL;
    }
}

struct TapeOff {
    size_t hin, geo, rbuf, pp0, x1;
    size_t s_in[OARD_MAX_LAYERS + 1], vec_in[OARD_MAX_LAYERS + 1];
    size_t agg[OARD_MAX_LAYERS], s_mid[OARD_MAX_LAYERS];
    size_t s_a[OARD_MAX_LAYERS], vec_a[OARD_MAX_LAYERS];
    size_t ew[OARD_MAX_LAYERS + 1];
    size_t z1[OARD_MAX_LAYERS], z2[OARD_MAX_LAYERS], att[OARD_MAX_LAYERS], z3[OARD_MAX_LAYERS];
    size_t zd1[OARD_MAX_LAYERS], cd[OARD_MAX_LAYERS];
    size_t total;
};
static TapeOff make_tape(const oard_config* c, const TopoDev& td) {
    const RDims d(c->hidden, c->num_radial);
    const size_t N = td.N, E = td.E + 1, A = td.A + 1;
    TapeOff t;
    memset(&t, 0, sizeof(t));
    size_t cur = 0;
    auto take = [&](size_t bytes) { size_t o = cur; cur = align_up(cur + bytes, 256); return o; };
    t.hin = take(N * 16 * 4); t.geo = take(A * GEO_STRIDE * 4); t.rbuf = take(A * d.RP * 4); t.pp0 = take(N * 4); t.x1 = take(N * 3 * 4);
    for (int l = 0; l <= c->num_layers; ++l) {
        t.s_in[l] = take(N * d.HP * 4); t.vec_in[l] = take(N * 3 * d.HP * 4); t.ew[l] = take(E * d.WP * 4);
        if (l == c->num_layers) break;
        t.agg[l] = take(N * d.HP * 4); t.s_mid[l] = take(N * d.HP * 4);
        t.s_a[l] = take(N * d.HP * 4); t.vec_a[l] = take(N * 3 * d.HP * 4);
        t.z1[l] = take(E * d.HP * 4); t.z2[l] = take(E * d.HP * 4); t.att[l] = take(E * 4); t.z3[l] = take(E * d.WP * 4);
        t.zd1[l] = take(A * d.D1P * 4); t.cd[l] = take(A * 3 * d.HP * 4);
    }
    t.total = cur;
    return t;
}

template <class D>
static int forward_impl(const oard_config* c, const TopoPart* topo, const float* wb, const float* const* xh,
                        const float* t, int t_scalar, const float* cond, float* const* out, char* ws, char* tape,
                        int* status, hipStream_t st) {
    const TopoDev& tp = topo->d;
    const PackOff po = make_layout(c);
    const WsOff w = make_ws(c, tp);
    const bool train = tape != nullptr;
    const TapeOff to = train ? make_tape(c, tp) : TapeOff{};
    const int emb = embed_dim(c);
    float* pos = (float*)(ws + w.pos); double* pf64 = (double*)(ws + w.pf64); float* pf32 = (float*)(ws + w.pf32);
    auto slot = [&](size_t ws_off, size_t tape_off) -> float* { return train ? (float*)(tape + tape_off) : (float*)(ws + ws_off); };
    float* x1 = slot(w.x1, to.x1); float* pp0 = slot(w.pp0, to.pp0); int* labels = (int*)(ws + w.labels);
    float* hin = slot(w.hin, to.hin); float* zemb = (float*)(ws + w.zemb); float* nb = (float*)(ws + w.nb);
    float* s = (float*)(ws + w.s); float* s1 = (float*)(ws + w.s1); float* ne1 = (float*)(ws + w.ne1);
    float* xhb = (float*)(ws + w.xh); float* P = (float*)(ws + w.P); float* Q = (float*)(ws + w.Q);
    float* xq = (float*)(ws + w.xq); float* vec = slot(w.vec, to.vec_in[0]); float* v2buf = (float*)(ws + w.v2buf);
    float* scal = (float*)(ws + w.sc0); float* vdot = (float*)(ws + w.vdot);
    float* geo = slot(w.geo, to.geo); double* d64 = (double*)(ws + w.d64); float* rbuf = slot(w.rbuf, to.rbuf);
    float* mbuf = (float*)(ws + w.mbuf); float* xmsg = (float*)(ws + w.xmsg);
    float* vmsg = (float*)(ws + w.vmsg); float* dpos = (float*)(ws + w.dpos); float* hout = (float*)(ws + w.hout);
    t_small = (w.small_a && !train) ? SmallScratch{(float*)(ws + w.small_a), (float*)(ws + w.small_b)} : SmallScratch{nullptr, nullptr};
    auto ew_at = [&](int l) -> float* { return train ? (float*)(tape + to.ew[l]) : (float*)(ws + w.ew); };
    float* ew = ew_at(0);
    auto s_at = [&](int l) -> float* { return train ? (float*)(tape + to.s_in[l]) : s; };
    auto s_mid_at = [&](int l) -> float* { return train ? (float*)(tape + to.s_mid[l]) : s; };

    ObjPtrs op;
    memset(&op, 0, sizeof(op));
    for (int k = 0; k < c->n_obj; ++k) {
        op.xh[k] = xh[k]; op.out[k] = out[k]; op.node_nf[k] = c->node_nf[k]; op.enc[k] = po.enc[k]; op.dec[k] = po.dec[k];
    }
    const long long N = tp.N, E = tp.E, A = tp.A;
    const unsigned gN = (unsigned)cdiv(N, 64), gE = (unsigned)cdiv(E, 64), gA = (unsigned)cdiv(A, 64);
    const double cutoff = (double)c->cutoff;
    const int gcl_variant = train ? 2 : g_gcl_variant, equi_variant = train ? 2 : g_equi_variant;
    const int node_variant = train ? 1 : g_node_variant;
    const bool gcl_skip = train || g_gcl_skip;
    const int stop_after = train ? 0 : g_stop_after;
    const bool use_al = !train && g_equi_skip && A > 0 && equi_variant != 0 && node_variant == 1;
    int* al_cnt = (int*)(ws + w.al_cnt);
    const ActList al = use_al ? ActList{(const int*)(ws + w.al_rows), (const int*)(ws + w.al_src), (const int*)(ws + w.al_pre), (const int*)(ws + w.al_n)}
                              : ActList{nullptr, nullptr, nullptr, nullptr};
    if (!use_al) HIP_TRY(hipMemsetAsync(ws + w.al_n, 0xff, sizeof(int), st));
    LAUNCH(F_OTHER, k_prep, cdiv(N, 128), 128, st, tp, op, wb, pos, hin, t, t_scalar, cond,
           c->condition_nf > 0 ? c->condition_nf : 0, c->condition_time, emb);
    LAUNCH(F_INIT, k_geom, tp.n_groups, 64, st, tp, (const float*)pos, cutoff, pf64, pf32, x1, pp0, labels);
    if (!(gcl_skip && gcl_variant != 0) || stop_after == 1)
        LAUNCH(F_INIT, k_fill_edges, std::min<long long>(cdiv((E - A + 1) * (D::WP / 4), 256), 8192), 256, st,
               wb + po.c0row, ew + (size_t)A * D::WP, E - A + 1, D::WP);
    if (A > 0) {
        LAUNCH(F_INIT, k_edge_geo, cdiv(A, 256), 256, st, tp, (const float*)pos, (const double*)pf64, cutoff, geo, d64, use_al ? al_cnt : nullptr);
        if (use_al) LAUNCH(F_INIT, k_active_list, cdiv(A, 256), 256, st, tp, (const float*)geo, (const int*)al_cnt, (int*)al.rows, (int*)al.src, (int*)al.pre, (int*)al.n);
        LAUNCH(F_INIT, k_rbf, cdiv(A * D::RP, 256), 256, st, tp, (const double*)d64, (const float*)geo,
               wb + po.rbf_means, wb + po.rbf_betas, cutoff, rbuf, ew, D::R, D::RP, D::H, D::WP);
    }
    LAUNCH(F_INIT, (k_node_embed<D>), gN, 256, st, tp, wb, po, (const float*)hin, zemb, nb);
    if (A > 0) LAUNCH(F_INIT, (k_radial_lin<D>), gA, 256, st, tp, wb, po, (const float*)rbuf, (const float*)geo, ew);
    constexpr int NW = D::HT <= 16 ? D::HT : 8;
    const unsigned gNb = (unsigned)cdiv(N, tp.npb);
    if (node_variant >= 1) {
        LAUNCH(F_INIT, (k_neighbor_v1<D, NW>), gNb, NW * 64, st, tp, wb, po, (const float*)zemb, (const float*)nb, (const float*)ew, s_at(0), s1);
        LAUNCH(F_INIT, (k_s2v_agg_v1<D, NW>), gNb, NW * 64, st, tp, (const float*)s1, (const float*)ew, (const float*)geo, ne1);
    } else if constexpr (kV0) {
        LAUNCH(F_INIT, (k_neighbor<D>), gN, 256, st, tp, wb, po, (const float*)zemb, (const float*)nb, (const float*)ew, s_at(0), s1);
        LAUNCH(F_INIT, (k_s2v_agg<D>), gN, 256, st, tp, (const float*)s1, (const float*)ew, (const float*)geo, ne1);
    } else return OARD_EINVAL;
    if (A > 0) LAUNCH2(F_INIT, (k_scalarize<D>), gA, (gA * topo->conc <= 2048 ? D::HT : 1), 256, st, tp, wb, po, (const float*)ne1, (const float*)geo, ew);
    HIP_TRY(hipMemsetAsync(vec, 0, (size_t)N * 3 * D::HP * sizeof(float), st));
    if (stop_after == 1) return OARD_OK;

    float* vec2 = (float*)(ws + w.vec2);
    float* vcur = vec;
    float* vnext = vec2;
    for (int l = 0; l < c->num_layers; ++l) {
        const LayerOff lo = po.layer[l];
        const bool nv1 = node_variant == 1 && equi_variant != 0;
        const unsigned gN16 = (unsigned)cdiv(N, tp.npb);
        float* ew_in = ew_at(l);
        float* ew_out = ew_at(l + 1);
        if (train) vnext = (float*)(tape + to.vec_in[l + 1]);

        if (nv1) LAUNCH(F_NODE, (k_node_pre_v1<D, NW>), gN16, NW * 64, st, tp, wb, po, lo, (const float*)s_at(l), (const float*)pp0, xhb, P, Q);
        else if constexpr (kV0) LAUNCH(F_NODE, (k_node_pre<D>), gN, 256, st, tp, wb, po, lo, (const float*)s, (const float*)pp0, xhb, P, Q);
        else return OARD_EINVAL;
        if (E > 0) {
            if (gcl_variant == 0) {
                if constexpr (kV0) LAUNCH(F_GCL_EDGE, (k_gcl_edge<D>), gE, 256, st, tp, wb, lo, (const float*)P, (const float*)Q, ew_in, mbuf);
                else return OARD_EINVAL;
            } else {
                GclTape gt{};
                if (train) gt = GclTape{(float*)(tape + to.z1[l]), (float*)(tape + to.z2[l]), (float*)(tape + to.att[l]), (float*)(tape + to.z3[l])};
                int rc = launch_gcl_v1<D>(c->precision, gcl_variant, topo->conc, tp, wb, lo, wb + lo.gcl_stream, P, Q, wb + po.u0, wb + po.c0row, l == 0,
                                          l == c->num_layers - 1, ew_in, ew_out, mbuf, train ? &gt : nullptr, st);
                if (rc != OARD_OK) return rc;
            }
        }
        const bool rows = tp.npb <= 4;
        if (nv1 && rows) LAUNCH(F_NODE, (k_gcl_node_v1<D, NW, true>), gN16, NW * 64, st, tp, wb, lo, (const float*)xhb, (const float*)mbuf, s_mid_at(l), xq,
                                train ? (float*)(tape + to.agg[l]) : nullptr);
        else if (nv1) LAUNCH(F_NODE, (k_gcl_node_v1<D, NW, false>), gN16, NW * 64, st, tp, wb, lo, (const float*)xhb, (const float*)mbuf, s_mid_at(l), xq,
                             train ? (float*)(tape + to.agg[l]) : nullptr);
        else if constexpr (kV0) LAUNCH(F_NODE, (k_gcl_node<D>), gN, 256, st, tp, wb, lo, (const float*)xhb, (const float*)mbuf, s, xq);
        else return OARD_EINVAL;
        if (stop_after == 100 + 10 * l + 1) { topo->vec_final = (size_t)((char*)vcur - ws); return OARD_OK; }
        if (equi_variant == 0) {
            if constexpr (kV0) {
                if (A > 0) LAUNCH(F_EQUI_EDGE, (k_equi_edge<D>), gA, 256, st, tp, wb, lo, (const float*)ew_out, (const float*)rbuf,
                                  (const float*)geo, (const float*)xq, (const float*)vcur, xmsg, vmsg);
                LAUNCH(F_NODE, (k_equi_agg<D>), gN, 256, st, tp, wb, lo, (const float*)xmsg, (const float*)vmsg, (const float*)x1,
                       s, vcur, v2buf, scal, vdot);
            } else return OARD_EINVAL;
        } else {
            const bool l0_skip = l == 0 && !train && g_equi_l0_skip && A > 0 && nv1 && !rows &&
                                 equi_v1_shape(c->precision, equi_variant, topo->conc, A, (const float*)(ws + w.d1s)) == 2;
            if (l == 0) g_equi_l0_taken = l0_skip;
            if (A > 0) {
                int rc = launch_equi_v1<D>(c->precision, equi_variant, topo->conc, tp, wb, lo, wb + lo.equi_stream, wb + lo.dp0b, ew_out, rbuf, vmsg,
                                           train ? (float*)(tape + to.zd1[l]) : nullptr, train ? (float*)(tape + to.cd[l]) : nullptr, st,
                                           (float*)(ws + w.d1s), al, l0_skip);
                if (rc != OARD_OK) return rc;
            }
#define EQUI_NODE_V1(D_, ROWS_, XC_) LAUNCH(F_NODE, (k_equi_node_v1<D_, NW, ROWS_, XC_>), gN16, NW * 64, st, tp, wb, lo, (const float*)vmsg, \
                       (const float*)xq, (const float*)geo, (const float*)x1, (const float*)s_mid_at(l), s_at(l + 1), (const float*)vcur, vnext, \
                       train ? (float*)(tape + to.s_a[l]) : nullptr, train ? (float*)(tape + to.vec_a[l]) : nullptr, al)
            if (nv1 && rows) {
                if (lo.xcross) EQUI_NODE_V1(D, true, true); else EQUI_NODE_V1(D, true, false);
            } else if (nv1 && l0_skip) {
                if (lo.xcross) EQUI_NODE_V1(Layer0<D>, false, true); else EQUI_NODE_V1(Layer0<D>, false, false);
            } else if (nv1) {
                if (lo.xcross) EQUI_NODE_V1(D, false, true); else EQUI_NODE_V1(D, false, false);
            } else if constexpr (kV0) {
                LAUNCH(F_NODE, (k_equi_agg_v1<D>), gN, 256, st, tp, wb, lo, (const float*)vmsg, (const float*)xq,
                       (const float*)geo, (const float*)x1, s, (const float*)vcur, vnext, v2buf, scal, vdot);
            } else return OARD_EINVAL;
            std::swap(vcur, vnext);
        }
        if constexpr (kV0) {
            if (!nv1) LAUNCH(F_NODE, (k_equi_upd<D>), gN, 256, st, tp, wb, lo, (const float*)scal, (const float*)vdot,
                             (const float*)v2buf, s, vcur);
        }
        if (stop_after == 100 + 10 * l + 2) { topo->vec_final = (size_t)((char*)vcur - ws); return OARD_OK; }
    }
    if (!train) topo->vec_final = (size_t)((char*)vcur - ws);
    if (train) {
        ZeroRows z;
        z.count = 0;
        auto add = [&](size_t off, size_t row, int ld) {
            if (z.count == 64) { LAUNCH(F_OTHER, k_zero_rows, 64, 256, st, z); z.count = 0; }
            z.p[z.count] = (float*)(tape + off) + row * (size_t)ld; z.n[z.count] = ld; ++z.count;
        };
        for (int l = 0; l <= c->num_layers; ++l) {
            add(to.ew[l], (size_t)E, D::WP);
            if (l == c->num_layers) break;
            add(to.z1[l], (size_t)E, D::HP); add(to.z2[l], (size_t)E, D::HP); add(to.att[l], (size_t)E, 1); add(to.z3[l], (size_t)E, D::WP);
            add(to.zd1[l], (size_t)A, D::D1P); add(to.cd[l], (size_t)A, 3 * D::HP);
        }
        add(to.geo, (size_t)A, GEO_STRIDE); add(to.rbuf, (size_t)A, D::RP);
        if (z.count > 0) LAUNCH(F_OTHER, k_zero_rows, z.count, 256, st, z);
    }
    if (node_variant >= 1)
        LAUNCH(F_NODE, (k_out_v1<D, NW>), gNb, NW * 64, st, tp, wb, po, (const float*)s_at(c->num_layers), (const float*)vcur, dpos, hout, status);
    else if constexpr (kV0)
        LAUNCH(F_NODE, (k_out<D>), gN, 256, st, tp, wb, po, (const float*)s, (const float*)vcur, dpos, hout, status);
    else return OARD_EINVAL;
    LAUNCH(F_OTHER, k_post, cdiv(N, 128), 128, st, tp, op, wb, (const float*)dpos, (const float*)hout, emb);
    HIP_TRY(hipGetLastError());
    return OARD_OK;
}

template <class F> static int dispatch_dims(const oard_config* c, F&& f) {
#define X(h, r) if (c->hidden == (h) && c->num_radial == (r)) { f(Dims<(h), (r)>{}); return 0; }
    OARD_DIMS_LIST
#undef X
    return OARD_EINVAL;
}
#define DISPATCH_DIMS(c, CALL)                                                                         \
    do {                                                                                               \
        if (dispatch_dims((c), [&](auto d_) { using D = decltype(d_); CALL; }) != 0) return OARD_EINVAL; \
    } while (0)

struct BwdLayerOff { size_t gcl, equi, watt; };
struct BwdOff { BwdLayerOff layer[OARD_MAX_LAYERS]; size_t total; };
// ... 404 lines not shown
        return OARD_EHIP;
    }
    *stage_out = stage;
    return OARD_OK;
}
static void topo_touch(const oard_topology* tp, hipStream_t st) {
    if (!tp) return;
    for (int i = 0; i < tp->n_used; ++i) if (tp->used_on[i] == st) return;
    if (tp->ready) (void)hipStreamWaitEvent(st, tp->ready, 0);
    if (tp->n_used < 4) tp->used_on[tp->n_used++] = st; else tp->used_many = true;
}

static int build_part(const oard_config* c, const int64_t* cm, const int64_t* nfs, int N_all, const std::vector<int>& obj_start,
                      const std::vector<int>& dense, const std::vector<long long>& ref_ptr_ref, int lo, int hi,
                      TopoPart& part, int& max_group, int& max_ns) {
    const int n_obj = c->n_obj, B = hi - lo;
    std::vector<int> order;
    for (int i = 0; i < N_all; ++i) if (dense[i] >= lo && dense[i] < hi) order.push_back(i);
    std::stable_sort(order.begin(), order.end(), [&](int a, int b) {
        if (dense[a] != dense[b]) return dense[a] < dense[b];
        return nfs[a] < nfs[b];
    });
    const int N = (int)order.size();
    if (N < 1) return OARD_EINVAL;
    std::vector<int> node_obj(N), node_row(N), node_ref(N), node_tidx(N), node_sample(N), sample_ptr(B + 1, 0),
        grp_ptr((size_t)B * n_obj + 1, 0), edge_ptr(N), act_ptr(N + 1, 0);
    for (int n = 0; n < N; ++n) {
        const int r = order[n], sb = dense[r] - lo;
        node_ref[n] = r; node_obj[n] = (int)nfs[r]; node_row[n] = r - obj_start[nfs[r]];
        node_tidx[n] = (int)cm[r]; node_sample[n] = sb;
        sample_ptr[sb + 1]++;
        grp_ptr[(size_t)sb * n_obj + nfs[r] + 1]++;
    }
    for (int b = 0; b < B; ++b) sample_ptr[b + 1] += sample_ptr[b];
    for (size_t q = 0; q < (size_t)B * n_obj; ++q) grp_ptr[q + 1] += grp_ptr[q];
    long long E = 0, A = 0;
    for (int b = 0; b < B; ++b) {
        const long long ns = sample_ptr[b + 1] - sample_ptr[b];
        max_ns = std::max(max_ns, (int)ns);
        for (int n = sample_ptr[b]; n < sample_ptr[b + 1]; ++n) { edge_ptr[n] = (int)E; E += ns - 1; }
        if (E > 0x7fffffffLL) return OARD_EINVAL;
    }
    for (size_t q = 0; q < (size_t)B * n_obj; ++q) {
        const long long ng = grp_ptr[q + 1] - grp_ptr[q];
        max_group = std::max(max_group, (int)ng);
        A += ng * (ng - 1);
    }
    if (max_group > OARD_MAX_GROUP || A > 0x7fffffffLL) return OARD_EINVAL;
    std::vector<int> edge_src((size_t)E + 1, 0), edge_tgt((size_t)E + 1, 0);
    for (int b = 0; b < B; ++b) {
        const int s0 = sample_ptr[b], s1 = sample_ptr[b + 1];
        for (int n = s0; n < s1; ++n) {
            size_t e = (size_t)edge_ptr[n];
            for (int m = s0; m < s1; ++m) if (m != n) { edge_src[e] = n; edge_tgt[e] = m; ++e; }
        }
    }
    std::vector<int> act_src((size_t)A + 1, 0), act_tgt((size_t)A + 1, 0), act_edge((size_t)A + 1, (int)E);
    {
        size_t a = 0;
        for (int n = 0; n < N; ++n) {
            const int q = node_sample[n] * n_obj + node_obj[n];
            const int g0 = grp_ptr[q], g1 = grp_ptr[q + 1], s0 = sample_ptr[node_sample[n]];
            act_ptr[n] = (int)a;
            for (int m = g0; m < g1; ++m) if (m != n) {
                act_src[a] = m; act_tgt[a] = n;
                act_edge[a] = edge_ptr[m] + (n - s0) - (n > m ? 1 : 0);
                ++a;
            }
        }
        act_ptr[N] = (int)a;
    }
    std::vector<int> edge_row((size_t)std::max<long long>(E, 1), -1), row_src((size_t)E + 1, 0), row_tgt((size_t)E + 1, 0),
        row_eid((size_t)E + 1, (int)E);
    {
        for (long long a = 0; a < A; ++a) {
            edge_row[act_edge[a]] = (int)a; row_src[a] = act_src[a]; row_tgt[a] = act_tgt[a]; row_eid[a] = act_edge[a];
        }
        long long r = A;
        for (long long e = 0; e < E; ++e)
            if (edge_row[e] < 0) { edge_row[e] = (int)r; row_src[r] = edge_src[e]; row_tgt[r] = edge_tgt[e]; row_eid[r] = (int)e; ++r; }
    }
    std::vector<long long> ref_edge_ptr(N);
    for (int n = 0; n < N; ++n) ref_edge_ptr[n] = ref_ptr_ref[node_ref[n]];

    std::vector<UploadItem> items;
    size_t cur = 0;
    auto add = [&](const void* p, size_t bytes) { UploadItem it{p, bytes, cur}; cur = align_up(cur + bytes, 256); items.push_back(it); return it.off; };
    const size_t o_obj = add(node_obj.data(), N * 4), o_row = add(node_row.data(), N * 4), o_ref = add(node_ref.data(), N * 4),
                 o_tidx = add(node_tidx.data(), N * 4), o_smp = add(node_sample.data(), N * 4),
                 o_sptr = add(sample_ptr.data(), (B + 1) * 4), o_eptr = add(edge_ptr.data(), N * 4),
                 o_esrc = add(edge_src.data(), edge_src.size() * 4), o_etgt = add(edge_tgt.data(), edge_tgt.size() * 4),
                 o_gptr = add(grp_ptr.data(), grp_ptr.size() * 4), o_aptr = add(act_ptr.data(), (N + 1) * 4),
                 o_asrc = add(act_src.data(), act_src.size() * 4), o_atgt = add(act_tgt.data(), act_tgt.size() * 4),
                 o_aedge = add(act_edge.data(), act_edge.size() * 4), o_rptr = add(ref_edge_ptr.data(), N * 8),
                 o_erow = add(edge_row.data(), edge_row.size() * 4), o_rsrc = add(row_src.data(), row_src.size() * 4),
                 o_rtgt = add(row_tgt.data(), row_tgt.size() * 4), o_reid = add(row_eid.data(), row_eid.size() * 4);
    size_t cap = 0;
    char* dev = (char*)pool_alloc(cur, &cap);
    if (!dev) return OARD_EHIP;
    if (int rc = pool_upload(dev, items, cur, &part.stage, &part.stage_cap)) { pool_release(dev, cap, nullptr, 0, false); return rc; }
    part.dev_cap = cap;
    part.dev_block = dev;
    TopoDev& d = part.d;
    d.N = N; d.B = B; d.n_obj = n_obj; d.n_groups = B * n_obj; d.E = E; d.A = A;
    d.node_obj = (const int*)(dev + o_obj); d.node_row = (const int*)(dev + o_row); d.node_ref = (const int*)(dev + o_ref);
    d.node_tidx = (const int*)(dev + o_tidx); d.node_sample = (const int*)(dev + o_smp); d.sample_ptr = (const int*)(dev + o_sptr);
    d.edge_ptr = (const int*)(dev + o_eptr); d.edge_src = (const int*)(dev + o_esrc); d.edge_tgt = (const int*)(dev + o_etgt);
    d.grp_ptr = (const int*)(dev + o_gptr); d.act_ptr = (const int*)(dev + o_aptr); d.act_src = (const int*)(dev + o_asrc);
    d.act_tgt = (const int*)(dev + o_atgt); d.act_edge = (const int*)(dev + o_aedge);
    d.ref_edge_ptr = (const long long*)(dev + o_rptr);
    d.edge_row = (const int*)(dev + o_erow); d.row_src = (const int*)(dev + o_rsrc); d.row_tgt = (const int*)(dev + o_rtgt);
    d.row_eid = (const int*)(dev + o_reid);
    return OARD_OK;
}

int oard_topology_create(const oard_config* c, const int64_t* cm, const int64_t* nfs, int64_t n_nodes,
                         oard_topology** out) {
    return oard_topology_create_parts(c, cm, nfs, n_nodes, g_parts, out);
}

int oard_topology_create_parts(const oard_config* c, const int64_t* cm, const int64_t* nfs, int64_t n_nodes,
                               int parts, oard_topology** out) {
    if (!config_ok(c) || !cm || !nfs || !out || n_nodes < 1 || n_nodes > (1 << 24)) return OARD_EINVAL;
    const int N = (int)n_nodes, n_obj = c->n_obj;
    std::vector<int> obj_start(n_obj + 1, 0);
    for (int i = 0; i < N; ++i) {
        if (nfs[i] < 0 || nfs[i] >= n_obj) return OARD_EINVAL;
        if (i > 0 && nfs[i] < nfs[i - 1]) return OARD_EINVAL;
        obj_start[nfs[i] + 1]++;
    }
    for (int k = 0; k < n_obj; ++k) obj_start[k + 1] += obj_start[k];
    std::vector<int64_t> samples(cm, cm + N);
    std::sort(samples.begin(), samples.end());
    samples.erase(std::unique(samples.begin(), samples.end()), samples.end());
    const int B = (int)samples.size();
    if (samples.front() < 0 || samples.back() > (1 << 30)) return OARD_EINVAL;
    std::vector<int> dense(N), ns_of(B, 0);
    for (int i = 0; i < N; ++i) {
        dense[i] = (int)(std::lower_bound(samples.begin(), samples.end(), cm[i]) - samples.begin());
        ns_of[dense[i]]++;
    }
    std::vector<long long> ref_ptr_ref(N);
    long long E_all = 0;
    for (int r = 0; r < N; ++r) { ref_ptr_ref[r] = E_all; E_all += ns_of[dense[r]] - 1; }

    int n_parts = parts > 0 ? parts : (B >= 32 ? 4 : (B >= 16 ? 2 : 1));
    n_parts = std::max(1, std::min(std::min(n_parts, OARD_MAX_PARTS), B));
    oard_topology* tp = new oard_topology();
    (void)hipGetDevice(&tp->device);
    tp->n_obj = n_obj; tp->B = B; tp->n_parts = n_parts;
    {
        std::vector<int> tab(2 * (size_t)N), seen(B, 0);
        for (int r = 0; r < N; ++r) { tab[r] = dense[r]; tab[(size_t)N + r] = seen[dense[r]]++; }
        const size_t b_int = 2 * (size_t)N * sizeof(int), b_all = align_up(b_int, 8) + (size_t)N * sizeof(long long);
        tp->ref_block = pool_alloc(b_all, &tp->ref_cap);
        if (!tp->ref_block) { delete tp; return OARD_EHIP; }
        const std::vector<UploadItem> ref_items = {{tab.data(), b_int, 0}, {ref_ptr_ref.data(), (size_t)N * sizeof(long long), align_up(b_int, 8)}};
        if (int rc = pool_upload(tp->ref_block, ref_items, b_all, &tp->ref_stage, &tp->ref_stage_cap)) { oard_topology_destroy(tp); return rc; }
        tp->ref_sample = (const int*)tp->ref_block; tp->ref_rank = tp->ref_sample + N;
        tp->ref_ptr = (const long long*)((char*)tp->ref_block + align_up(b_int, 8));
        tp->N_ref = N;
    }
    for (int k = 0; k <= n_obj && k <= OARD_MAX_OBJECTS; ++k) tp->obj_start[k] = obj_start[k];
    for (int p = 0; p < n_parts; ++p) {
        const int lo = (int)((long long)B * p / n_parts), hi = (int)((long long)B * (p + 1) / n_parts);
        int rc = build_part(c, cm, nfs, N, obj_start, dense, ref_ptr_ref, lo, hi, tp->parts[p], tp->max_group, tp->max_ns);
        if (rc != OARD_OK) { oard_topology_destroy(tp); return rc; }
        tp->N += tp->parts[p].d.N; tp->E += tp->parts[p].d.E; tp->A += tp->parts[p].d.A;
        tp->parts[p].conc = n_parts;
    }
    {
        const int npb = g_npb > 0 ? g_npb : (int)std::max<long long>(1, std::min<long long>(16, cdiv(tp->N, 256)));
        for (int p = 0; p < n_parts; ++p) tp->parts[p].d.npb = npb;
    }
    if (n_parts > 1) {
        HIP_TRY(hipEventCreateWithFlags(&tp->ev_fork, hipEventDisableTiming));
        for (int p = 1; p < n_parts; ++p) {
            tp->side[p] = device_streams()[(p - 1) % 3];
            if (!tp->side[p]) { oard_topology_destroy(tp); return OARD_EHIP; }
            HIP_TRY(hipEventCreateWithFlags(&tp->ev_join[p], hipEventDisableTiming));
        }
    }
    HIP_TRY(hipEventCreateWithFlags(&tp->ready, hipEventDisableTiming));
    HIP_TRY(hipEventRecord(tp->ready, device_streams()[2]));
    *out = tp;
    return OARD_OK;
}

void oard_topology_destroy(oard_topology* tp) {
    if (!tp) return;
    int cur = tp->device;
    (void)hipGetDevice(&cur);
    if (cur != tp->device) (void)hipSetDevice(tp->device);
    struct Restore { int cur, dev; ~Restore() { if (cur != dev) (void)hipSetDevice(cur); } } restore_{cur, tp->device};
    for (int p = 0; p < OARD_MAX_PARTS; ++p) {
// ... 791 lines not shown
    return OARD_OK;
}

int oard_adamw_step_dev(float* param, const float* grad, float* exp_avg, float* exp_avg_sq, float* max_exp_avg_sq, int64_t n, double lr,
                        double beta1, double beta2, double eps, double weight_decay, int amsgrad, int clip, double* clip_state,
                        int capacity, const float* grad_norm, const float* flag, float* out4, oard_stream_t stream) {
    if (!param || !grad || !exp_avg || !exp_avg_sq || (amsgrad && !max_exp_avg_sq) || n < 0 || !clip_state || capacity < 1 || capacity > 64 ||
        !grad_norm || !flag || !out4)
        return OARD_EINVAL;
    LAUNCH(F_OTHER, k_clip_decide, 1, 64, (hipStream_t)stream, clip_state, capacity, grad_norm, flag, clip, lr, beta1, beta2, eps, weight_decay, out4);
    if (n > 0)
        LAUNCH(F_OTHER, k_adamw_dev, cdiv(n, 256), 256, (hipStream_t)stream, param, grad, exp_avg, exp_avg_sq, max_exp_avg_sq, (long long)n, amsgrad,
               reinterpret_cast<const AdamScal*>(clip_state + 4 + capacity));
    HIP_TRY(hipGetLastError());
    return OARD_OK;
}

int oard_train_scratch_entry(const oard_config* c, const oard_topology* topo, int which, size_t* offset_bytes, int64_t* rows,
                             int64_t* row_floats) {
    if (!config_ok(c) || !topo || topo->n_parts != 1 || !offset_bytes || !rows || !row_floats) return OARD_EINVAL;
    const TopoDev& d = topo->parts[0].d;
    const TrainWs w = make_train_ws(c, d);
    const RDims r(c->hidden, c->num_radial);
    switch (which) {
        case OARD_SCRATCH_XH: *offset_bytes = w.xh; *rows = d.N; *row_floats = r.HP; break;
        case OARD_SCRATCH_XQ: *offset_bytes = w.xq; *rows = d.N; *row_floats = 3 * r.HP; break;
        case OARD_SCRATCH_CR: *offset_bytes = w.cr; *rows = d.A + 1; *row_floats = 3 * r.HP; break;
        case OARD_SCRATCH_DCD: *offset_bytes = w.dcd; *rows = d.A + 1; *row_floats = 3 * r.HP; break;
        case OARD_SCRATCH_DCR: *offset_bytes = w.dcr; *rows = d.A + 1; *row_floats = 3 * r.HP; break;
        default: return OARD_EINVAL;
    }
    return OARD_OK;
}

int oard_tap(const oard_config* c, const oard_topology* topo, const void* ws_, int which, int layer, float* dst,
             oard_stream_t stream) {
    topo_touch(topo, (hipStream_t)stream);
    if (!config_ok(c) || !topo || !ws_ || !dst || layer != 0) return OARD_EINVAL;
    const RDims d(c->hidden, c->num_radial);
    ws_total(c, topo);
    hipStream_t st = (hipStream_t)stream;
    for (int p = 0; p < topo->n_parts; ++p) {
        const TopoDev& tp = topo->parts[p].d;
        const WsOff w = make_ws(c, tp);
        const char* ws = (const char*)ws_ + topo->parts[p].ws_off;
        auto nodes = [&](const float* src, int ld, int sections, int sect_pad, int sect_len) {
            const long long tot = (long long)tp.N * sections * sect_len;
            hipLaunchKernelGGL(k_tap_nodes, dim3((unsigned)cdiv(tot, 256)), dim3(256), 0, st, tp, src, ld, sections, sect_pad, sect_len, dst);
        };
        switch (which) {
            case OARD_TAP_S: nodes((const float*)(ws + w.s), d.HP, 1, d.HP, d.H); break;
            case OARD_TAP_VEC: nodes((const float*)(ws + topo->parts[p].vec_final), 3 * d.HP, 3, d.HP, d.H); break;
            case OARD_TAP_NE1: nodes((const float*)(ws + w.ne1), 3 * d.HP, 3, d.HP, d.H); break;
            case OARD_TAP_POS_FRAME: nodes((const float*)(ws + w.pf32), 3, 1, 3, 3); break;
            case OARD_TAP_DPOS: nodes((const float*)(ws + w.dpos), 3, 1, 3, 3); break;
            case OARD_TAP_HOUT: nodes((const float*)(ws + w.hout), 16, 1, 16, c->in_hidden); break;
            case OARD_TAP_LABELS:
                hipLaunchKernelGGL(k_tap_labels, dim3((unsigned)cdiv(tp.N, 256)), dim3(256), 0, st, tp, (const int*)(ws + w.labels), dst);
                break;
            case OARD_TAP_EDGE:
                if (tp.E > 0)
                    hipLaunchKernelGGL(k_tap_edges, dim3((unsigned)cdiv(tp.E * d.W, 256)), dim3(256), 0, st, tp,
                                       (const float*)(ws + w.ew), d.WP, d.W, dst);
                break;
            default: return OARD_EINVAL;
        }
    }
    HIP_TRY(hipGetLastError());
    return OARD_OK;
}

int oard_debug_stop_after(int code) { g_stop_after = code; return OARD_OK; }
int oard_debug_option(const char* name, int value) {
    if (!name) return OARD_EINVAL;
    if (!kV0 && value == 0 && (strcmp(name, "gcl_variant") == 0 || strcmp(name, "equi_variant") == 0 || strcmp(name, "node_variant") == 0))
        return OARD_EINVAL;
    if (strcmp(name, "gcl_variant") == 0) { g_gcl_variant = value; return OARD_OK; }
    if (strcmp(name, "equi_variant") == 0) { g_equi_variant = value; return OARD_OK; }
    if (strcmp(name, "node_variant") == 0) { g_node_variant = value; return OARD_OK; }
    if (strcmp(name, "experiments") == 0) return kV0 ? OARD_OK : OARD_EINVAL;
    if (strcmp(name, "gcl_skip") == 0) { g_gcl_skip = value; return OARD_OK; }
    if (strcmp(name, "equi_skip") == 0) { g_equi_skip = value; return OARD_OK; }
    if (strcmp(name, "equi_l0_skip") == 0) { g_equi_l0_skip = value; return OARD_OK; }
    if (strcmp(name, "equi_l0_taken") == 0) return g_equi_l0_taken ? OARD_OK : OARD_EINVAL;
    if (strcmp(name, "gcl_persist") == 0) { g_gcl_persist = value; return OARD_OK; }
    if (strcmp(name, "gcl_grid") == 0) { g_gcl_grid = value; return OARD_OK; }
    if (strcmp(name, "skip_families") == 0) { g_skip_families = value; return OARD_OK; }
    if (strcmp(name, "parts") == 0) { g_parts = value; return OARD_OK; }
    if (strcmp(name, "sequential") == 0) { g_sequential = value; return OARD_OK; }
    if (strcmp(name, "poison") == 0) { g_poison = value; return OARD_OK; }
    if (strcmp(name, "auto_small") == 0) { g_auto_small = value; return OARD_OK; }
    if (strcmp(name, "auto_tiny") == 0) { g_auto_tiny = value; return OARD_OK; }
    if (strcmp(name, "npb") == 0) { g_npb = value; return OARD_OK; }
    if (strcmp(name, "wgrad_wgs") == 0) { g_wgrad_wgs = value; return OARD_OK; }
    if (strcmp(name, "wgrad_t16") == 0) { g_wgrad_t16 = value; return OARD_OK; }
    if (strcmp(name, "wgrad_queue") == 0) { g_wgrad_queue = value; return OARD_OK; }
    if (strcmp(name, "gate_fold") == 0) { g_gate_fold = value; return OARD_OK; }
    if (strcmp(name, "wgrad_lds") == 0) { g_wgrad_lds = value; return OARD_OK; }
    if (strcmp(name, "wgrad_shapes") == 0) { g_wgrad_shapes = value & 3; return OARD_OK; }
    if (strcmp(name, "train_dual") == 0) { g_train_dual = value; return OARD_OK; }
    if (strcmp(name, "small_split") == 0) { g_small_split = value; return OARD_OK; }
    return OARD_EINVAL;
}
#ifdef OARD_PHASE_PROBE
int oard_debug_probe_read(unsigned long long* out8) {
    if (!out8) return OARD_EINVAL;
    HIP_TRY(hipDeviceSynchronize());
    HIP_TRY(hipMemcpyFromSymbol(out8, HIP_SYMBOL(g_phase_probe), 8 * sizeof(unsigned long long)));
    unsigned long long z[8] = {};
    HIP_TRY(hipMemcpyToSymbol(HIP_SYMBOL(g_phase_probe), z, sizeof(z)));
    return OARD_OK;
}
#endif
#ifdef OARD_TIMELINE
int oard_debug_timeline_read(long long* out, int waves) {
    if (!out || waves < 1 || waves > 16) return OARD_EINVAL;
    HIP_TRY(hipDeviceSynchronize());
    HIP_TRY(hipMemcpyFromSymbol(out, HIP_SYMBOL(g_timeline), (size_t)waves * TL_MAX * sizeof(long long)));
    return OARD_OK;
}
#endif
#ifdef OARD_EXPERIMENTS
int oard_debug_fp_timeouts(unsigned int* out) {
    if (!out) return OARD_EINVAL;
    HIP_TRY(hipDeviceSynchronize());
    HIP_TRY(hipMemcpyFromSymbol(out, HIP_SYMBOL(g_fp_timeouts), sizeof(unsigned int)));
    return OARD_OK;
}
#endif
int oard_timing_enable(int on) { g_timing.on = on != 0; return OARD_OK; }
int oard_timing_reset(void) {
    g_timing.flush();
    for (int f = 0; f < F_COUNT; ++f) { g_timing.total_ms[f] = 0; g_timing.launches[f] = 0; }
    return OARD_OK;
}
int oard_timing_get(const char* family, double* total_ms, int64_t* launches) {
    if (!family || !total_ms || !launches) return OARD_EINVAL;
    g_timing.flush();
    for (int f = 0; f < F_COUNT; ++f)
        if (strcmp(family, kFamilyNames[f]) == 0) { *total_ms = g_timing.total_ms[f]; *launches = g_timing.launches[f]; return OARD_OK; }
    return OARD_EINVAL;
}

}
```

### oareactdiff_amd/csrc/oard_inst.h

```cpp
#pragma once
#if !defined(OARD_EXPERIMENTS) && !defined(OARD_SINGLE_TU)

#define OARD_UNPAREN(...) __VA_ARGS__
#ifdef OARD_INST_DEFINE
#define OARD_INST(K, ARGS) template __global__ void OARD_UNPAREN K ARGS;
#else
#define OARD_INST(K, ARGS) extern template __global__ void OARD_UNPAREN K ARGS;
#endif
#ifndef OARD_DIMS_LIST
#define OARD_DIMS_LIST X(196, 96) X(32, 8) X(32, 32)
#endif
#define OARD_BOOL4(M, D) M(D, true, true) M(D, false, true) M(D, true, false) M(D, false, false)

#define OARD_NW(h) (((h) + 15) / 16 <= 16 ? ((h) + 15) / 16 : 8)
#define OARD_A_GCL (TopoDev, const float*, const float*, const float*, const float*, const float*, long long, long long, const float*, float*, float*, GclTape)

#if !defined(OARD_INST_DEFINE) || defined(OARD_INST_UNIT_GCL_P)
#define OARD_I_GCL_P(D, S1, S3) OARD_INST((k_gcl_edge_p<OARD_UNPAREN D, S1, S3, false>), OARD_A_GCL) OARD_INST((k_gcl_edge_p<OARD_UNPAREN D, S1, S3, true>), OARD_A_GCL)
#define X(h, r) OARD_BOOL4(OARD_I_GCL_P, (Dims<h, r>))
OARD_DIMS_LIST
#undef X
#endif

#if !defined(OARD_INST_DEFINE) || defined(OARD_INST_UNIT_GCL_V1)
#define OARD_I_GCL_V1(D, S1, S3) \
    OARD_INST((k_gcl_edge_v1<OARD_UNPAREN D, 8, 2, S1, S3, false, 2, 3>), OARD_A_GCL) OARD_INST((k_gcl_edge_v1<OARD_UNPAREN D, 8, 2, S1, S3, true, 2, 3>), OARD_A_GCL) \
    OARD_INST((k_gcl_edge_v1<OARD_UNPAREN D, 4, 2, S1, S3, false, 2, 2>), OARD_A_GCL) \
    OARD_INST((k_gcl_edge_small<OARD_UNPAREN D, 8, S1, S3>), (TopoDev, const float*, LayerOff, const float*, const float*, const float*, const float*, long long, long long, float*, float*))
#define X(h, r) OARD_BOOL4(OARD_I_GCL_V1, (Dims<h, r>))
OARD_DIMS_LIST
#undef X
#endif

#if !defined(OARD_INST_DEFINE) || defined(OARD_INST_UNIT_B3)
#define OARD_A_EQUI_B3 (TopoDev, const float*, const float*, const float*, const float*, const float*, float*, float*, float*, float*, ActList)
#define OARD_I_GCL_B3(D, S1, S3) OARD_INST((k_gcl_edge_b3<OARD_UNPAREN D, S1, S3, false>), OARD_A_GCL) OARD_INST((k_gcl_edge_b3<OARD_UNPAREN D, S1, S3, true>), OARD_A_GCL)
#define X(h, r) OARD_BOOL4(OARD_I_GCL_B3, (Dims<h, r>)) OARD_INST((k_equi_edge_b3<Dims<h, r>, false>), OARD_A_EQUI_B3) OARD_INST((k_equi_edge_b3<Dims<h, r>, true>), OARD_A_EQUI_B3)
OARD_DIMS_LIST
#undef X
#endif

#if !defined(OARD_INST_DEFINE) || defined(OARD_INST_UNIT_EQUI)
#define OARD_A_EQUI (TopoDev, const float*, const float*, const float*, const float*, float*, float*, float*, ActList, int)
#define OARD_A_EQUI_NODE (TopoDev, const float*, LayerOff, const float*, const float*, const float*, const float*, const float*, float*, const float*, float*, float*, float*, ActList)
#define X(h, r) \
    OARD_INST((k_equi_edge_v1<Dims<h, r>, 8, false>), OARD_A_EQUI) OARD_INST((k_equi_edge_v1<Dims<h, r>, 8, true>), OARD_A_EQUI) \
    OARD_INST((k_equi_edge_v1<Dims<h, r>, 4, false>), OARD_A_EQUI) \
    OARD_INST((k_equi_node_v1<Dims<h, r>, OARD_NW(h), false, false>), OARD_A_EQUI_NODE) OARD_INST((k_equi_node_v1<Dims<h, r>, OARD_NW(h), false, true>), OARD_A_EQUI_NODE) \
    OARD_INST((k_equi_node_v1<Dims<h, r>, OARD_NW(h), true, false>), OARD_A_EQUI_NODE) OARD_INST((k_equi_node_v1<Dims<h, r>, OARD_NW(h), true, true>), OARD_A_EQUI_NODE) \
    OARD_INST((k_equi_node_v1<Layer0<Dims<h, r> >, OARD_NW(h), false, false>), OARD_A_EQUI_NODE) OARD_INST((k_equi_node_v1<Layer0<Dims<h, r> >, OARD_NW(h), false, true>), OARD_A_EQUI_NODE) \
    OARD_INST((k_gcl_edge_bwd<Dims<h, r>, 8, 2, true>), (TopoDev, const float*, long long, long long, GclBwdArgs)) \
    OARD_INST((k_gcl_edge_bwd<Dims<h, r>, 8, 2, false>), (TopoDev, const float*, long long, long long, GclBwdArgs)) \
    OARD_INST((k_equi_edge_bwd<Dims<h, r>, 8>), (TopoDev, const float*, const float*, const float*, float*, float*))
OARD_DIMS_LIST
#undef X
#endif

#if !defined(OARD_INST_DEFINE) || defined(OARD_INST_UNIT_NODE)
#define OARD_A_GCL_NODE (TopoDev, const float*, LayerOff, const float*, const float*, float*, float*, float*)
#define OARD_A_OUT (TopoDev, const float*, PackOff, const float*, const float*, float*, float*, int*)
#define OARD_A_SCAL_BWD (TopoDev, const float*, const float*, int, const float*, const float*, float*, float*)
#define OARD_A_MSG_BWD (TopoDev, const float*, Strided3, Strided3, const float*, Strided3, const float*, int, Strided3, float*, float*, float*, float*, int, int, int)
#define X(h, r) \
    OARD_INST((k_gcl_node_v1<Dims<h, r>, OARD_NW(h), false>), OARD_A_GCL_NODE) OARD_INST((k_gcl_node_v1<Dims<h, r>, OARD_NW(h), true>), OARD_A_GCL_NODE) \
    OARD_INST((k_out_v1<Dims<h, r>, OARD_NW(h)>), OARD_A_OUT) \
    OARD_INST((k_scalarize_bwd<Dims<h, r>, 2, false>), OARD_A_SCAL_BWD) OARD_INST((k_scalarize_bwd<Dims<h, r>, 2, true>), OARD_A_SCAL_BWD) \
    OARD_INST((k_equi_msg_bwd<Dims<h, r> >), OARD_A_MSG_BWD)
OARD_DIMS_LIST
#undef X
OARD_INST((k_lin3u_bwd_fused<4>), (const float*, const float*, const float*, long long, float*, float*))
#define OARD_I_ROWS(KB, EPI) OARD_INST((k_rows_dense<KB, EPI, 8>), (RowsDense)) OARD_INST((k_rows_dense_long<KB, EPI, 8, 4>), (RowsDense))
OARD_I_ROWS(13, 0) OARD_I_ROWS(13, 2) OARD_I_ROWS(13, 3) OARD_I_ROWS(7, 3) OARD_I_ROWS(6, 0) OARD_I_ROWS(6, 1) OARD_I_ROWS(4, 1) OARD_I_ROWS(4, 3)
OARD_INST((k_rows_dense<26, 1, 8>), (RowsDense)) OARD_INST((k_rows_dense<26, 3, 8>), (RowsDense))
OARD_INST((k_rows_dense2<13, 1, 8, 13>), (RowsDense2)) OARD_INST((k_rows_dense2<13, 2, 8, 13>), (RowsDense2))
OARD_INST((k_rows_dense2<26, 1, 8, 13>), (RowsDense2)) OARD_INST((k_rows_dense2<39, 2, 8, 13>), (RowsDense2))
#endif

#if !defined(OARD_INST_DEFINE) || defined(OARD_INST_UNIT_WGRAD)
#define OARD_A_WG (const float*, int, int, const float*, int, int, long long, long long, long long, int, int, float*, float*, float*)
OARD_INST((k_wgrad_t16<4, 7, false>), (WgtArgs)) OARD_INST((k_wgrad_t16<4, 7, true>), (WgtArgs)) OARD_INST((k_wgrad_t16<5, 3, false>), (WgtArgs))
OARD_INST((k_wgrad_t16<5, 5, true>), (WgtArgs)) OARD_INST((k_wgrad_t16<5, 7, true>), (WgtArgs)) OARD_INST((k_wgrad_t16<6, 5, false>), (WgtArgs))
OARD_INST((k_wgrad_t16<6, 7, false>), (WgtArgs))
OARD_INST((k_wgrad<false, 7>), OARD_A_WG) OARD_INST((k_wgrad<false, 8>), OARD_A_WG) OARD_INST((k_wgrad<true, 7>), OARD_A_WG) OARD_INST((k_wgrad<true, 8>), OARD_A_WG)
OARD_INST((k_wgrad_lds<false, 7, 4, 2>), OARD_A_WG) OARD_INST((k_wgrad_lds<false, 8, 4, 2>), OARD_A_WG)
OARD_INST((k_wgrad_lds<true, 7, 4, 2>), OARD_A_WG) OARD_INST((k_wgrad_lds<true, 8, 4, 2>), OARD_A_WG)
#endif

#endif
```

### oareactdiff_amd/csrc/oard_layout.h

```cpp
#pragma once
#include <hip/hip_runtime.h>
#include <stdint.h>
#include <stddef.h>
#include "../../include/oard.h"

#define OARD_MAX_LAYERS 16
#define OARD_MAX_GROUP 1024

template <int H_, int R_>
struct Dims {
    static constexpr int H = H_, R = R_;
    static constexpr int HT = (H + 15) / 16, HP = HT * 16;
    static constexpr int W = 3 * H + R, WB = (W + 15) / 16, WP = WB * 16;
    static constexpr int RB = (R + 15) / 16, RP = RB * 16;
    static constexpr int H2 = H / 2, PB = (H2 + 15) / 16, PP = PB * 16;
    static constexpr int D1T = (3 * H + 15) / 16, D1P = D1T * 16;
    static constexpr int H4 = H / 4;
    static_assert(H % 4 == 0 && R % 4 == 0, "feature widths must be multiples of 4");
};

struct RDims {
    int H, R, HT, HP, W, WB, WP, RB, RP, H2, PB, PP, D1T, D1P, H4;
    explicit RDims(int h, int r) {
        H = h; R = r; HT = (H + 15) / 16; HP = HT * 16; W = 3 * H + R; WB = (W + 15) / 16; WP = WB * 16;
        RB = (R + 15) / 16; RP = RB * 16; H2 = H / 2; PB = (H2 + 15) / 16; PP = PB * 16;
        D1T = (3 * H + 15) / 16; D1P = D1T * 16; H4 = H / 4;
    }
};

#define L3T_X 16.0f
#define L3T_H 0.03125f
#define L3T_N 1024
#define L3T_FLOATS (2 * (L3T_N + 1) + 4)

struct LayerOff {
    size_t ln_g_w, ln_g_b, W1a, b1, W1b, W1c, W2, b2, watt, batt, W3, b3, nm0, nm0b, nm1, nm1b;
    size_t ln_q_w, ln_q_b, xp0, xp2, dp0, dp0b, dp2, dp2b, rbfp;
    size_t vp, xv0, xv2, l3u;
    size_t l3t;
    size_t gcl_stream, equi_stream;
    size_t gcl_b3, equi_b3;
    int xcross;
};
struct PackOff {
    size_t emb, emb_b, nbemb, nbemb_b, s2v, s2v_b, rl0, rl0_b, rl2, rl2_b;
    size_t lin3;
    size_t pe0;
    size_t pe1, embout, embout_b, v1p, v2p, un0, un0_b, un2, un2_b;
    size_t c0row;
    size_t u0;
    size_t rbf_means, rbf_betas;
    size_t enc[OARD_MAX_OBJECTS], dec[OARD_MAX_OBJECTS];
    LayerOff layer[OARD_MAX_LAYERS];
    size_t total;
    int signed_scal;
};

struct TopoDev {
    int N, B, n_obj, n_groups;
    int npb;
    long long E, A;
    const int *node_obj, *node_row, *node_ref, *node_tidx, *node_sample, *sample_ptr;
    const int *edge_ptr, *edge_src, *edge_tgt;
    const int *edge_row;
    const int *row_src, *row_tgt;
    const int *row_eid;
    const int *grp_ptr;
    const int *act_ptr, *act_src, *act_tgt, *act_edge;
    const long long *ref_edge_ptr;
};

struct ActList {
    const int* rows;
    const int* src;
    const int* pre;
    const int* n;
};

#define OARD_MAX_PARTS 8
struct TopoPart {
    TopoDev d;
    void* dev_block = nullptr;
    size_t dev_cap = 0;
    void* stage = nullptr;
    size_t stage_cap = 0;
    size_t ws_off = 0;
    int conc = 1;
    mutable size_t vec_final = 0;
};
struct oard_topology {
    int device = 0;
    int n_parts = 0;
    TopoPart parts[OARD_MAX_PARTS];
    int n_obj = 0, B = 0;
    long long N = 0, E = 0, A = 0;
    int max_group = 0, max_ns = 0;
    int obj_start[OARD_MAX_OBJECTS + 1] = {};
    hipStream_t side[OARD_MAX_PARTS] = {};
    hipEvent_t ev_fork = nullptr, ev_join[OARD_MAX_PARTS] = {};
    void* ref_block = nullptr;
    size_t ref_cap = 0;
    void* ref_stage = nullptr;
    size_t ref_stage_cap = 0;
    hipEvent_t ready = nullptr;
    mutable hipStream_t used_on[4] = {};
    mutable int n_used = 0;
    mutable bool used_many = false;
    const int *ref_sample = nullptr, *ref_rank = nullptr;
    const long long* ref_ptr = nullptr;
    int N_ref = 0;
};

struct WsOff {
    size_t pos, pf64, pf32, x1, pp0, labels, hin, zemb, nb, s, s1, ne1, xh, P, Q, xq, vec, vec2, v2buf, sc0, vdot,
        geo, d64, rbuf, ew, mbuf, xmsg, vmsg, dpos, hout, total;
    size_t al_rows, al_src, al_pre, al_cnt, al_n;
    size_t d1s;
    size_t small_a, small_b;
};
```

### oareactdiff_amd/csrc/oard_node_v1.h

```cpp
#pragma once
#include "oard_kernels.h"

OARD_DEV f4 lds_blk(const float* v, int b, int lane) { return *reinterpret_cast<const f4*>(v + b * 256 + lane * 4); }
OARD_DEV void lds_st(float* v, int t, int lane, f4 x) { *reinterpret_cast<f4*>(v + t * 256 + lane * 4) = x; }

#ifndef OARD_NODE_PF
#define OARD_NODE_PF 13
#endif
template <int KB>
OARD_DEV f4 dense_tile_lds(const float* __restrict__ wp, int t, const float* in, int lane, f4 init) {
    const float* base = wp + ((size_t)t * KB * 64 + lane) * 4;
    f4 c0 = init, c1 = f4zero();
    constexpr int G = OARD_NODE_PF;
#pragma unroll
    for (int b0 = 0; b0 < KB; b0 += G) {
        f4 a[G];
#pragma unroll
        for (int i = 0; i < G; ++i)
            if (b0 + i < KB) a[i] = ld_f4(base + (size_t)(b0 + i) * 256);
        __builtin_amdgcn_sched_barrier(0);
#pragma unroll
        for (int i = 0; i < G; ++i)
            if (b0 + i < KB) {
                const f4 x = lds_blk(in, b0 + i, lane);
// ... 181 lines not shown
    r.L = npb == 1 ? 16 : (npb == 2 ? 8 : 4); r.npb = npb;
    const int e = lane & 15;
    r.node = e / r.L; r.slot = e % r.L;
    r.live = r.node < npb && blockIdx.x * npb + r.node < N;
    return r;
}
OARD_DEV float rows_total(float x, const RowLanes& r, int lane) {
    for (int d = 1; d < r.L; d <<= 1) x += __shfl_xor(x, d, 64);
    const int e = lane & 15;
    return __shfl(x, (lane & 48) | ((e < r.npb ? e : 0) * r.L), 64);
}
OARD_DEV f4 rows_total4(f4 v, const RowLanes& r, int lane) {
    return (f4){rows_total(v.x, r, lane), rows_total(v.y, r, lane), rows_total(v.z, r, lane), rows_total(v.w, r, lane)};
}

template <class D, int WAVES>
__global__ __launch_bounds__(WAVES * 64) void k_node_pre_v1(TopoDev tp, const float* __restrict__ wb, PackOff po,
                                                            LayerOff lo, const float* __restrict__ s,
                                                            const float* __restrict__ pp0, float* __restrict__ xh,
                                                            float* __restrict__ P, float* __restrict__ Q) {
    __shared__ __attribute__((aligned(16))) float sm[(D::PB + 2 * D::HT) * 256];
    float* hid = sm;
    float* sv = sm + D::PB * 256;
    float* xv = sv + D::HT * 256;
    const NodeBlk nb = node_blk(tp.N, tp.npb);
    const float pp = pp0[nb.n];
    for (int b = nb.wave; b < D::PB; b += WAVES) {
        const int k0 = 16 * b + 4 * nb.g;
        const float* w = wb + po.pe0;
        f4 h;
        h.x = k0 + 0 < D::H2 ? silu1(w[(k0 + 0) * 3] * pp) : 0.f;
        h.y = k0 + 1 < D::H2 ? silu1(w[(k0 + 1) * 3] * pp) : 0.f;
        h.z = k0 + 2 < D::H2 ? silu1(w[(k0 + 2) * 3] * pp) : 0.f;
        h.w = k0 + 3 < D::H2 ? silu1(w[(k0 + 3) * 3] * pp) : 0.f;
        lds_st(hid, b, nb.lane, h);
    }
    __syncthreads();
    constexpr int TPW = (D::HT + WAVES - 1) / WAVES, TPW2 = (2 * D::HT + WAVES - 1) / WAVES;
    {
        TileJob job[TPW];
        f4 acc[TPW];
#pragma unroll
        for (int i = 0; i < TPW; ++i) {
            const int t = min(nb.wave + i * WAVES, D::HT - 1);
            job[i] = tile_job<D::PB>(wb + po.pe1, t, hid);
            acc[i] = f4zero();
        }
        dense_seq<D::PB, TPW, OARD_NODE_PRE_G>(job, nb.lane, acc);
#pragma unroll
        for (int i = 0; i < TPW; ++i)
            if (nb.wave + i * WAVES < D::HT)
                lds_st(sv, nb.wave + i * WAVES, nb.lane, ld_blk(s, nb.n, D::HP, nb.wave + i * WAVES, nb.lane) + acc[i]);
    }
    __syncthreads();
    float mean, rstd;
    ln_stats_lds<D::HT, D::H>(sv, nb.lane, mean, rstd);
    for (int t = nb.wave; t < D::HT; t += WAVES) {
        const f4 y = ln_apply<D::H>(lds_blk(sv, t, nb.lane), mean, rstd, wb + lo.ln_g_w, wb + lo.ln_g_b, t, nb.lane);
        lds_st(xv, t, nb.lane, y);
        if (nb.valid) st_blk(xh, nb.n, D::HP, t, nb.lane, y);
    }
    __syncthreads();
    {
        TileJob job[TPW2];
        f4 acc[TPW2];
#pragma unroll
        for (int i = 0; i < TPW2; ++i) {
            const int t = min(nb.wave + i * WAVES, 2 * D::HT - 1);
            job[i] = t < D::HT ? tile_job<D::HT>(wb + lo.W1a, t, xv) : tile_job<D::HT>(wb + lo.W1b, t - D::HT, xv);
            acc[i] = t < D::HT ? ld_vec(wb + lo.b1, t, nb.lane) : f4zero();
        }
        dense_seq<D::HT, TPW2, OARD_NODE_PRE_G>(job, nb.lane, acc);
#pragma unroll
        for (int i = 0; i < TPW2; ++i) {
            const int t = nb.wave + i * WAVES;
            if (t < 2 * D::HT && nb.valid) {
                if (t < D::HT) st_blk(P, nb.n, D::HP, t, nb.lane, acc[i]);
                else st_blk(Q, nb.n, D::HP, t - D::HT, nb.lane, acc[i]);
            }
        }
    }
}

template <class D, int WAVES, bool ROWS = false>
__global__ __launch_bounds__(WAVES * 64) void k_gcl_node_v1(TopoDev tp, const float* __restrict__ wb, LayerOff lo,
                                                            const float* __restrict__ xh, const float* __restrict__ mbuf,
                                                            float* __restrict__ s, float* __restrict__ xq,
                                                            float* __restrict__ agg_out ) {
    __shared__ __attribute__((aligned(16))) float sm[4 * D::HT * 256];
    float* in = sm;
    float* hm = sm + 2 * D::HT * 256;
    float* sv = sm + 3 * D::HT * 256;
    const NodeBlk nb = node_blk(tp.N, tp.npb);
    const int smp = tp.node_sample[nb.n];
    const int deg = nb.valid ? tp.sample_ptr[smp + 1] - tp.sample_ptr[smp] - 1 : 0;
    const size_t e0 = (size_t)tp.edge_ptr[nb.n];
    const int mx = wave_max(deg);
    const float inv = 1.0f / (float)max(deg, 1);
    for (int t = nb.wave; t < D::HT; t += WAVES) {
        lds_st(in, t, nb.lane, ld_blk(xh, nb.n, D::HP, t, nb.lane));
        f4 a0 = f4zero(), a1 = f4zero();
        if (ROWS) {
            const RowLanes rl = row_lanes(tp.N, tp.npb, nb.lane);
            const int nn = min(blockIdx.x * tp.npb + rl.node, tp.N - 1);
            const int smp2 = tp.node_sample[nn];
            const int deg2 = rl.live ? tp.sample_ptr[smp2 + 1] - tp.sample_ptr[smp2] - 1 : 0;
            const size_t e2 = (size_t)tp.edge_ptr[nn];
            const int mx2 = wave_max(deg2), last2 = max(deg2 - 1, 0);
            for (int k = 0; k < mx2; k += 2 * rl.L) {
                const int k0 = k + rl.slot, k1 = k0 + rl.L;
                const f4 r0 = ld_blk(mbuf, e2 + min(k0, last2), D::HP, t, nb.lane), r1 = ld_blk(mbuf, e2 + min(k1, last2), D::HP, t, nb.lane);
                if (k0 < deg2) a0 += r0;
                if (k1 < deg2) a1 += r1;
            }
            a0 = rows_total4(a0 + a1, rl, nb.lane);
            a1 = f4zero();
        }
        const int last = max(deg - 1, 0);
        for (int k = 0; !ROWS && k < mx; k += 8) {
            f4 r[8];
#pragma unroll
            for (int i = 0; i < 8; ++i) r[i] = ld_blk(mbuf, e0 + min(k + i, last), D::HP, t, nb.lane);
#pragma unroll
            for (int i = 0; i < 8; ++i) {
                const f4 v = k + i < deg ? r[i] : f4zero();
                if (i & 1) a1 += v; else a0 += v;
            }
        }
        lds_st(in, D::HT + t, nb.lane, (a0 + a1) * inv);
        if (agg_out != nullptr && nb.valid) st_blk(agg_out, nb.n, D::HP, t, nb.lane, (a0 + a1) * inv);
    }
    __syncthreads();
    constexpr int TPW = (D::HT + WAVES - 1) / WAVES, TPW3 = (3 * D::HT + WAVES - 1) / WAVES;
    int tw[TPW];
#pragma unroll
    for (int i = 0; i < TPW; ++i) tw[i] = min(nb.wave + i * WAVES, D::HT - 1);
    {
        TileJob job[TPW];
        f4 acc[TPW];
#pragma unroll
        for (int i = 0; i < TPW; ++i) { job[i] = tile_job<2 * D::HT>(wb + lo.nm0, tw[i], in); acc[i] = ld_vec(wb + lo.nm0b, tw[i], nb.lane); }
        dense_seq<2 * D::HT, TPW, OARD_GCL_NODE_G>(job, nb.lane, acc);
#pragma unroll
        for (int i = 0; i < TPW; ++i)
            if (nb.wave + i * WAVES < D::HT) lds_st(hm, tw[i], nb.lane, silu4(acc[i]));
    }
    __syncthreads();
    {
        TileJob job[TPW];
        f4 acc[TPW];
#pragma unroll
        for (int i = 0; i < TPW; ++i) { job[i] = tile_job<D::HT>(wb + lo.nm1, tw[i], hm); acc[i] = ld_vec(wb + lo.nm1b, tw[i], nb.lane); }
        dense_seq<D::HT, TPW, OARD_GCL_NODE_G>(job, nb.lane, acc);
#pragma unroll
        for (int i = 0; i < TPW; ++i)
            if (nb.wave + i * WAVES < D::HT) {
                const f4 v = lds_blk(in, tw[i], nb.lane) + acc[i];
                lds_st(sv, tw[i], nb.lane, v);
                if (nb.valid) st_blk(s, nb.n, D::HP, tw[i], nb.lane, v);
            }
    }
    __syncthreads();
    float mean, rstd;
    ln_stats_lds<D::HT, D::H>(sv, nb.lane, mean, rstd);
    float* xln = in;
    float* hq = in + D::HT * 256;
    for (int t = nb.wave; t < D::HT; t += WAVES)
        lds_st(xln, t, nb.lane, ln_apply<D::H>(lds_blk(sv, t, nb.lane), mean, rstd, wb + lo.ln_q_w, wb + lo.ln_q_b, t, nb.lane));
    __syncthreads();
    {
        TileJob job[TPW];
        f4 acc[TPW];
#pragma unroll
        for (int i = 0; i < TPW; ++i) { job[i] = tile_job<D::HT>(wb + lo.xp0, tw[i], xln); acc[i] = f4zero(); }
        dense_seq<D::HT, TPW, OARD_GCL_NODE_G>(job, nb.lane, acc);
#pragma unroll
        for (int i = 0; i < TPW; ++i)
            if (nb.wave + i * WAVES < D::HT) lds_st(hq, tw[i], nb.lane, silu4(acc[i]));
    }
    __syncthreads();
    {
        TileJob job[TPW3];
        f4 acc[TPW3];
#pragma unroll
        for (int i = 0; i < TPW3; ++i) {
            job[i] = tile_job<D::HT>(wb + lo.xp2, min(nb.wave + i * WAVES, 3 * D::HT - 1), hq);
            acc[i] = f4zero();
        }
        dense_seq<D::HT, TPW3, OARD_GCL_NODE_G>(job, nb.lane, acc);
#pragma unroll
        for (int i = 0; i < TPW3; ++i)
            if (nb.wave + i * WAVES < 3 * D::HT && nb.valid) st_blk(xq, nb.n, 3 * D::HP, nb.wave + i * WAVES, nb.lane, acc[i]);
    }
}

OARD_DEV void lin3u_stage(const float* __restrict__ p, float* l3s, int tid, int nthreads) {
    for (int i = tid; i < 48 * 12; i += nthreads) {
        const int k = i / 12, j = i % 12;
        l3s[i] = j < 8 ? p[192 + j * 48 + k] : (j == 8 ? p[3 * k] : (j == 9 ? p[144 + k] : 0.f));
    }
}
OARD_DEV f4 lin3u4(const float* l3s, const float* __restrict__ p, f4 x) {
// ... 496 lines not shown
```

Before: 3613 reaction-steps/s.

## Segment-reduce GCL edge messages in-wave and gather partial sums in node kernel

Adds an MSUM mode where the GCL edge kernels walk a column ordering grouped by source node and reduce the message rows of same-source lanes with DPP row shifts. Only the segment head writes a partial sum, so mbuf shrinks from one row per edge to one per 16-lane segment, and the node kernel sums a few partials instead of every incoming edge row. This cuts the write and gather traffic for messages. In exchange it adds a host-built col_info/node_cols table, extra DPP work per tile, inline asm with hazard nops, and a separate path that training does not use. It is on by default.

After: 3662 reaction-steps/s, median of 6. +1.3%, better.

```diff
diff --git a/oareactdiff_amd/_capi.py b/oareactdiff_amd/_capi.py
--- a/oareactdiff_amd/_capi.py
+++ b/oareactdiff_amd/_capi.py
@@ -152,7 +152,7 @@
     L.oard_timing_reset.argtypes = []; L.oard_timing_reset.restype = C.c_int
     L.oard_timing_get.argtypes = [C.c_char_p, C.POINTER(C.c_double), C.POINTER(i64)]; L.oard_timing_get.restype = C.c_int
     for env, opt in (("OARD_GCL_VARIANT", b"gcl_variant"), ("OARD_EQUI_VARIANT", b"equi_variant"),
-                     ("OARD_NODE_VARIANT", b"node_variant"), ("OARD_GCL_SKIP", b"gcl_skip"), ("OARD_EQUI_SKIP", b"equi_skip"), ("OARD_EQUI_L0_SKIP", b"equi_l0_skip"), ("OARD_GCL_PERSIST", b"gcl_persist"), ("OARD_GCL_GRID", b"gcl_grid"), ("OARD_PARTS", b"parts"), ("OARD_SEQUENTIAL", b"sequential"), ("OARD_POISON", b"poison"), ("OARD_AUTO_SMALL", b"auto_small"), ("OARD_AUTO_TINY", b"auto_tiny"), ("OARD_NPB", b"npb"),
+                     ("OARD_NODE_VARIANT", b"node_variant"), ("OARD_GCL_SKIP", b"gcl_skip"), ("OARD_EQUI_SKIP", b"equi_skip"), ("OARD_EQUI_L0_SKIP", b"equi_l0_skip"), ("OARD_GCL_MSUM", b"gcl_msum"), ("OARD_GCL_PERSIST", b"gcl_persist"), ("OARD_GCL_GRID", b"gcl_grid"), ("OARD_PARTS", b"parts"), ("OARD_SEQUENTIAL", b"sequential"), ("OARD_POISON", b"poison"), ("OARD_AUTO_SMALL", b"auto_small"), ("OARD_AUTO_TINY", b"auto_tiny"), ("OARD_NPB", b"npb"),
                      ("OARD_WGRAD_WGS", b"wgrad_wgs"), ("OARD_WGRAD_LDS", b"wgrad_lds"), ("OARD_WGRAD_T16", b"wgrad_t16"), ("OARD_WGRAD_QUEUE", b"wgrad_queue"), ("OARD_GATE_FOLD", b"gate_fold"), ("OARD_WGRAD_SHAPES", b"wgrad_shapes"), ("OARD_TRAIN_DUAL", b"train_dual"), ("OARD_SMALL_SPLIT", b"small_split"),
                      ("OARD_SKIP_FAMILIES", b"skip_families")):
         if os.environ.get(env) not in (None, ""):
diff --git a/oareactdiff_amd/csrc/oard_edge_p.h b/oareactdiff_amd/csrc/oard_edge_p.h
--- a/oareactdiff_amd/csrc/oard_edge_p.h
+++ b/oareactdiff_amd/csrc/oard_edge_p.h
@@ -1,7 +1,7 @@
 #pragma once
 #include "oard_edge_v1.h"
 
-template <class D, bool DO_S1, bool DO_S3, bool TRAIN = false>
+template <class D, bool DO_S1, bool DO_S3, bool TRAIN = false, bool MSUM = false>
 __global__ __launch_bounds__(512, 2) void k_gcl_edge_p(TopoDev tp, const float* __restrict__ stream,
                                                        const float* __restrict__ P, const float* __restrict__ Q,
                                                        const float* __restrict__ u0, const float* __restrict__ c0,
@@ -15,6 +15,7 @@
     constexpr int P0 = DO_S1 ? 0 : S::NP1, PEND = DO_S3 ? S::NPH : S::NP1 + S::NP2, NPR = PEND - P0;
     static_assert(NPR >= DIST, "a round must be at least as long as the prefetch distance");
     static_assert(HT >= 2, "the phase barrier sits inside the first chain of a phase");
+    static_assert(!MSUM || !TRAIN, "the training-mode forward tapes agg from the per-edge message rows");
     constexpr int BAR_AT = OARD_BAR_AT < HT / 2 ? OARD_BAR_AT : HT / 2;
 
     const int lane = threadIdx.x & 63, g = lane >> 4;
@@ -30,6 +31,16 @@
         const int slot = is_half(r) ? wave - 4 : wave;
         const long long c = r0 + (((hb0 + 2 * r) << 2) + slot) * 16 + (lane & 15);
         return (size_t)((slot >= 0 && c < r1) ? c : tp.E);
+    };
+    auto col_of = [&](int r) -> long long {
+        return r0 + (((hb0 + 2 * r) << 2) + (is_half(r) ? wave - 4 : wave)) * 16 + (lane & 15);
+    };
+    auto info_of = [&](int r) -> i4 {
+        const int slot = is_half(r) ? wave - 4 : wave;
+        const long long c = col_of(r);
+        i4 ci = {(int)tp.E, 0, 0, -1};
+        if (slot >= 0 && c < r1) ci = *reinterpret_cast<const i4*>(tp.col_info + 4 * c);
+        return ci;
     };
 
     SlabPrefetch<WAVES, S::SLAB, 1, 1, RING> pf;
@@ -69,9 +80,10 @@
     float* orow = nullptr;
     f4 h1[HT];
     f4 xn[GP];
+    auto rd_row = [&](size_t row) -> size_t { return (MSUM && row == (size_t)tp.E) ? (size_t)tp.col_info[4 * r0] : row; };
     auto set_rows = [&](size_t row) {
         e = row;
-        erow = ew_in + e * D::WP + 4 * g;
+        erow = ew_in + rd_row(e) * D::WP + 4 * g;
         orow = ew_out + e * D::WP + 4 * g;
     };
     auto load_xn = [&](f4 (&x)[GP], const float* er) {
@@ -79,7 +91,7 @@
         for (int gg = 0; gg < GP; ++gg) x[gg] = (DO_S1 && gg < WB) ? ld_edge(er + 16 * gg) : f4zero();
     };
     size_t eid = 0;
-    int src = 0, tgt = 0;
+    int src = 0, tgt = 0, key = 0;
     auto load_h1 = [&]() {
 #pragma unroll
         for (int t = 0; t < HT; ++t) {
@@ -88,8 +100,8 @@
         }
     };
     if (active_in(0)) {
-        set_rows(row_of(0));
-        eid = (size_t)tp.row_eid[e]; src = tp.row_src[e]; tgt = tp.row_tgt[e];
+        if (MSUM) { const i4 ci = info_of(0); set_rows((size_t)ci.x); src = ci.y; tgt = ci.z; key = ci.w; }
+        else { set_rows(row_of(0)); eid = (size_t)tp.row_eid[e]; src = tp.row_src[e]; tgt = tp.row_tgt[e]; }
         load_h1();
         load_xn(xn, erow);
     }
@@ -107,6 +119,8 @@
         const bool nxt = more && active_in(r + 1);
         int src_n = 0, tgt_n = 0;
         size_t eid_n = 0;
+        i4 ci_n = {0, 0, 0, -1};
+        auto next_row = [&]() -> size_t { return (MSUM && DO_S3) ? (size_t)ci_n.x : row_of(r + 1); };
         f4 xn_n[GP];
         f4 hp[HT], hq[HT];
         int lp = P0;
@@ -221,8 +235,11 @@
                 if ((S::NP2 - 1) * GP + gg < HT) st_blk(tape.z2, e, D::HP, (S::NP2 - 1) * GP + gg, lane, pz2[gg]);
         }
         if (!DO_S3) {
-#pragma unroll
-            for (int t = 0; t < HT; ++t) st_blk(mbuf, eid, D::HP, t, lane, m[t]);
+            if (MSUM) st_msum<D>(mbuf, col_of(r), key, m, lane);
+            else {
+#pragma unroll
+                for (int t = 0; t < HT; ++t) st_blk(mbuf, eid, D::HP, t, lane, m[t]);
+            }
         } else {
             f4 pend[GP], pendz[TRAIN ? GP : 1];
             f4 om[GP];
@@ -230,8 +247,10 @@
                 constexpr bool LAST = decltype(last_tag)::value;
                 auto post = [&]() {
                     if (p3 == 0) {
-#pragma unroll
-                        for (int t = 0; t < HT; ++t) st_blk(mbuf, eid, D::HP, t, lane, m[t]);
+                        if (!MSUM) {
+#pragma unroll
+                            for (int t = 0; t < HT; ++t) st_blk(mbuf, eid, D::HP, t, lane, m[t]);
+                        }
                     } else {
 #pragma unroll
                         for (int gg = 0; gg < GP; ++gg) {
@@ -249,10 +268,13 @@
                     }
                     if (nxt) {
                         if (p3 == 0) {
-                            const size_t en = row_of(r + 1);
-                            src_n = tp.row_src[en]; tgt_n = tp.row_tgt[en]; eid_n = (size_t)tp.row_eid[en];
+                            if (MSUM) ci_n = info_of(r + 1);
+                            else {
+                                const size_t en = row_of(r + 1);
+                                src_n = tp.row_src[en]; tgt_n = tp.row_tgt[en]; eid_n = (size_t)tp.row_eid[en];
+                            }
                         }
-                        if (LAST) load_xn(xn_n, ew_in + row_of(r + 1) * D::WP + 4 * g);
+                        if (LAST) load_xn(xn_n, ew_in + rd_row(next_row()) * D::WP + 4 * g);
                     }
                 };
                 auto hook = [&]() { if (bar_left > 0 && --bar_left == 0) { PHASE_BARRIER(); post(); } pf.tick(); };
@@ -267,6 +289,7 @@
                     }
                 }
                 if (bar_left > 0) { bar_left = 0; PHASE_BARRIER(); post(); }
+                if (MSUM && p3 == 0) st_msum<D>(mbuf, col_of(r), key, m, lane);
                 pf.flush();
                 ++gp; ++lp;
             };
@@ -287,13 +310,15 @@
         }
 
         if (nxt) {
-            set_rows(row_of(r + 1));
+            if (MSUM && !DO_S3) ci_n = info_of(r + 1);
+            set_rows(MSUM ? (size_t)ci_n.x : row_of(r + 1));
+            if (MSUM) { src = ci_n.y; tgt = ci_n.z; key = ci_n.w; }
             if (DO_S3) {
-                eid = eid_n; src = src_n; tgt = tgt_n;
+                if (!MSUM) { eid = eid_n; src = src_n; tgt = tgt_n; }
 #pragma unroll
                 for (int gg = 0; gg < GP; ++gg) xn[gg] = xn_n[gg];
             } else {
-                eid = (size_t)tp.row_eid[e]; src = tp.row_src[e]; tgt = tp.row_tgt[e];
+                if (!MSUM) { eid = (size_t)tp.row_eid[e]; src = tp.row_src[e]; tgt = tp.row_tgt[e]; }
                 load_xn(xn, erow);
             }
             load_h1();
diff --git a/oareactdiff_amd/csrc/oard_edge_v1.h b/oareactdiff_amd/csrc/oard_edge_v1.h
--- a/oareactdiff_amd/csrc/oard_edge_v1.h
+++ b/oareactdiff_amd/csrc/oard_edge_v1.h
@@ -3,6 +3,7 @@
 
 typedef __attribute__((address_space(3))) void* lds_ptr_t;
 typedef const __attribute__((address_space(1))) void* gbl_ptr_t;
+typedef int i4 __attribute__((ext_vector_type(4)));
 
 OARD_DEV void glds16(const float* gsrc_lane, float* lds_chunk);
 OARD_DEV void glds16u(const float* chunk_uniform, unsigned lane_byte_off, float* lds_chunk) {
@@ -201,6 +202,45 @@
 OARD_DEV f4 ld_edge(const float* p) { return ld_f4(p); }
 #endif
 
+template <int CTRL>
+OARD_DEV float dpp_row(float x) {
+    return __builtin_bit_cast(float, __builtin_amdgcn_update_dpp(0, __builtin_bit_cast(int, x), CTRL, 0xf, 0xf, true));
+}
+template <int CTRL>
+OARD_DEV int dpp_row_i(int x) { return __builtin_amdgcn_update_dpp(0, x, CTRL, 0xf, 0xf, true); }
+struct SegLanes {
+    float k1, k2, k4, k8;
+    bool head;
+};
+OARD_DEV SegLanes seg_lanes(int key) {
+    SegLanes s;
+    s.k1 = dpp_row_i<0x101>(key) == key ? 1.f : 0.f; s.k2 = dpp_row_i<0x102>(key) == key ? 1.f : 0.f;
+    s.k4 = dpp_row_i<0x104>(key) == key ? 1.f : 0.f; s.k8 = dpp_row_i<0x108>(key) == key ? 1.f : 0.f;
+    const int prev = dpp_row_i<0x111>(key);
+    s.head = key > 0 && prev != key;
+    return s;
+}
+OARD_DEV f4 seg_sum(f4 v, const SegLanes& s) {
+#define OARD_SEG_STEP(k, d) \
+        "v_fmac_f32_dpp %0, %0, " k " row_shl:" d " row_mask:0xf bank_mask:0xf bound_ctrl:1\n\t" \
+        "v_fmac_f32_dpp %1, %1, " k " row_shl:" d " row_mask:0xf bank_mask:0xf bound_ctrl:1\n\t" \
+        "v_fmac_f32_dpp %2, %2, " k " row_shl:" d " row_mask:0xf bank_mask:0xf bound_ctrl:1\n\t" \
+        "v_fmac_f32_dpp %3, %3, " k " row_shl:" d " row_mask:0xf bank_mask:0xf bound_ctrl:1\n\t"
+    asm volatile("s_nop 4\n\t" OARD_SEG_STEP("%4", "1") OARD_SEG_STEP("%5", "2") OARD_SEG_STEP("%6", "4") OARD_SEG_STEP("%7", "8")
+                 : "+v"(v.x), "+v"(v.y), "+v"(v.z), "+v"(v.w) : "v"(s.k1), "v"(s.k2), "v"(s.k4), "v"(s.k8));
+#undef OARD_SEG_STEP
+    return v;
+}
+template <class D>
+OARD_DEV void st_msum(float* __restrict__ msum, long long col, int key, const f4 (&m)[D::HT], int lane) {
+    const SegLanes s = seg_lanes(key);
+#pragma unroll
+    for (int t = 0; t < D::HT; ++t) {
+        const f4 v = seg_sum(m[t], s);
+        if (s.head) st_blk(msum, (size_t)col, D::HP, t, lane, v);
+    }
+}
+
 template <class D, int GP>
 struct GclStream {
     static constexpr int HT = D::HT, WB = D::WB, G1 = HT, G2 = HT + 1, NG2 = HT + 1;
@@ -227,7 +267,7 @@
 #ifndef OARD_BAR_AT
 #define OARD_BAR_AT 2
 #endif
-template <class D, int WAVES, int GP, bool DO_S1, bool DO_S3, bool TRAIN, int MINW = 2, int RING = 2>
+template <class D, int WAVES, int GP, bool DO_S1, bool DO_S3, bool TRAIN, bool MSUM = false, int MINW = 2, int RING = 2>
 __global__ __launch_bounds__(WAVES * 64, MINW) void k_gcl_edge_v1(TopoDev tp, const float* __restrict__ stream,
                                                                const float* __restrict__ P, const float* __restrict__ Q,
                                                                const float* __restrict__ u0, const float* __restrict__ c0,
@@ -243,6 +283,7 @@
     TL_DECL
     TL(0);
     static_assert(RING == 2 || RING == 3, "two slabs (barrier at the phase start) or three (barrier inside the phase)");
+    static_assert(!MSUM || !TRAIN, "the training-mode forward tapes agg from the per-edge message rows");
     static_assert(RING == 2 || HT >= 2, "the phase barrier must sit inside the FIRST chain of a phase (S3 stores the previous phase's results behind it)");
     constexpr int DIST = RING - 1;
     constexpr int BAR_AT = OARD_BAR_AT < HT / 2 ? OARD_BAR_AT : HT / 2;
@@ -267,13 +308,18 @@
     auto SL = [&](int p) -> const float* { return smem + (size_t)slab_of(p) * S::SLAB * 256 + lane * 4; };
 
     const long long c = r0 + ((long long)blockIdx.x * WAVES + wave) * 16 + (lane & 15);
-    const size_t e = (size_t)(c < r1 ? c : tp.E);
-    const float* erow = ew_in + e * D::WP + 4 * g;
+    i4 ci = {0, 0, 0, -1};
+    if (MSUM && c < r1) ci = *reinterpret_cast<const i4*>(tp.col_info + 4 * c);
+    const size_t e = (size_t)(c < r1 ? (MSUM ? (long long)ci.x : c) : tp.E);
+    const size_t e_rd = (MSUM && e == (size_t)tp.E) ? (size_t)tp.col_info[4 * r0] : e;
+    const float* erow = ew_in + e_rd * D::WP + 4 * g;
     float* orow = ew_out + e * D::WP + 4 * g;
     f4 h1[HT];
-    const size_t eid = (size_t)tp.row_eid[e];
+    const size_t eid = MSUM ? 0 : (size_t)tp.row_eid[e];
+    int key = 0;
     {
-        const int src = tp.row_src[e], tgt = tp.row_tgt[e];
+        const int src = MSUM ? ci.y : tp.row_src[e], tgt = MSUM ? ci.z : tp.row_tgt[e];
+        if (MSUM) key = ci.w;
 #pragma unroll
         for (int t = 0; t < HT; ++t) {
             h1[t] = ld_blk(P, src, D::HP, t, lane) + ld_blk(Q, tgt, D::HP, t, lane);
@@ -391,8 +437,11 @@
             if ((S::NP2 - 1) * GP + gg < HT) st_blk(tape.z2, e, D::HP, (S::NP2 - 1) * GP + gg, lane, pz2[gg]);
     }
     if (!DO_S3) {
-#pragma unroll
-        for (int t = 0; t < HT; ++t) st_blk(mbuf, eid, D::HP, t, lane, m[t]);
+        if (MSUM) st_msum<D>(mbuf, c, key, m, lane);
+        else {
+#pragma unroll
+            for (int t = 0; t < HT; ++t) st_blk(mbuf, eid, D::HP, t, lane, m[t]);
+        }
         PROBE_END(pf);
         TL_END();
         return;
@@ -403,8 +452,10 @@
         auto post = [&]() {
             TL(1);
             if (p3 == 0) {
-#pragma unroll
-                for (int t = 0; t < HT; ++t) st_blk(mbuf, eid, D::HP, t, lane, m[t]);
+                if (!MSUM) {
+#pragma unroll
+                    for (int t = 0; t < HT; ++t) st_blk(mbuf, eid, D::HP, t, lane, m[t]);
+                }
             } else {
 #pragma unroll
                 for (int gg = 0; gg < GP; ++gg) {
@@ -437,6 +488,7 @@
         }
         TL(4);
         if (RING == 3 && bar_left > 0) { bar_left = 0; PHASE_BARRIER(); post(); }
+        if (MSUM && p3 == 0) st_msum<D>(mbuf, c, key, m, lane);
         pf.flush();
         ++p;
     };
diff --git a/oareactdiff_amd/csrc/oard_hip.hip b/oareactdiff_amd/csrc/oard_hip.hip
--- a/oareactdiff_amd/csrc/oard_hip.hip
+++ b/oareactdiff_amd/csrc/oard_hip.hip
@@ -69,6 +69,8 @@
 int g_npb = 0;
 int g_poison = 0;
 int g_equi_l0_skip = 1;
+int g_gcl_msum = 1;
+int g_gcl_msum_taken = 0;
 int g_equi_l0_taken = 0;
 int g_parts = 0;
 int g_small_split = 128;
@@ -303,7 +305,7 @@
     w.xq = take(N * 3 * d.HP * 4); w.vec = take(N * 3 * d.HP * 4); w.vec2 = take(N * 3 * d.HP * 4); w.v2buf = take(N * 3 * d.HP * 4);
     w.sc0 = take(N * d.HP * 4); w.vdot = take(N * d.HP * 4);
     w.geo = take(A * GEO_STRIDE * 4); w.d64 = take(A * 8); w.rbuf = take(A * d.RP * 4);
-    w.ew = take(E * d.WP * 4); w.mbuf = take(E * d.HP * 4);
+    w.ew = take(E * d.WP * 4); w.mbuf = take(std::max(E, (size_t)(td.CI + td.CX) + 1) * d.HP * 4);
     w.xmsg = take(A * d.HP * 4); w.vmsg = take(A * 3 * d.HP * 4);
     w.dpos = take(N * 3 * 4); w.hout = take(N * 16 * 4);
     w.al_rows = take(A * 4); w.al_src = take(A * 4); w.al_pre = take(A * 4); w.al_cnt = take((size_t)cdiv((long long)td.A, 256) * 4 + 4); w.al_n = take(4);
@@ -335,7 +337,7 @@
         LAUNCH_LDS(F_GCL_EDGE, (k_gcl_edge_v1<D, WV_, GP_, S1, S3, false>), cdiv(r1 - r0, 16 * WV_), WV_ * 64, \
                    (GclStream<D, GP_>::LDS_BYTES), st, tp, stream, P, Q, u0, c0, r0, r1, ew_in, ew_out, mbuf, GclTape{}); return OARD_OK; }
 #define GCL_RING3(TRAIN_, tape_) do { \
-        LAUNCH_LDS(F_GCL_EDGE, (k_gcl_edge_v1<D, 8, 2, S1, S3, TRAIN_, 2, 3>), cdiv(r1 - r0, 16 * 8), 8 * 64, \
+        LAUNCH_LDS(F_GCL_EDGE, (k_gcl_edge_v1<D, 8, 2, S1, S3, TRAIN_, false, 2, 3>), cdiv(r1 - r0, 16 * 8), 8 * 64, \
                    (GclStream<D, 2>::LDS_BYTES / 2 * 3), st, tp, stream, P, Q, u0, c0, r0, r1, ew_in, ew_out, mbuf, tape_); return OARD_OK; } while (0)
 static int device_cus() {
     static int cus[64] = {};
@@ -349,10 +351,17 @@
     }
     return cus[d];
 }
+static bool gcl_v1_throughput(int prec, int variant, int conc, long long cols) {
+    if (variant == 2 && cdiv(cols, 16) * conc <= 1024LL * g_auto_small) variant = 3;
+    if ((variant == 2 || variant == 3) && cdiv(cols, 16) * conc <= 512LL * g_auto_tiny) variant = 6;
+    return variant == 2 && !(prec & OARD_PREC_GCL_BF16X3);
+}
 template <class D, bool S1, bool S3>
 int launch_gcl_v1s(int prec, int variant, int conc, const TopoDev& tp, const float* wb, const LayerOff& lo, const float* stream, const float* P, const float* Q, const float* u0,
-                   const float* c0, long long r0, long long r1, const float* ew_in, float* ew_out, float* mbuf, const GclTape* tape, hipStream_t st) {
+                   const float* c0, long long r0, long long r1, const float* ew_in, float* ew_out, float* mbuf, const GclTape* tape, hipStream_t st,
+                   bool msum = false) {
     if (r1 <= r0) return OARD_OK;
+    if (msum && (tape || !gcl_v1_throughput(prec, variant, conc, r1 - r0))) return OARD_EINVAL;
     if (tape && (prec & OARD_PREC_TRAIN_BF16X3)) {
         LAUNCH_LDS(F_GCL_EDGE, (k_gcl_edge_b3<D, S1, S3, true>), cdiv(r1 - r0, 16 * 8), 8 * 64, (GclB3Stream<D>::LDS_BYTES), st, tp,
                    wb + lo.gcl_b3, P, Q, u0, c0, r0, r1, ew_in, ew_out, mbuf, *tape);
@@ -392,8 +401,18 @@
             if (g_gcl_persist > 1 || (g_gcl_persist == 1 && conc == 1)) {
                 const long long nhalf = cdiv(cdiv(r1 - r0, 16), 4);
                 const long long want = g_gcl_grid > 0 ? g_gcl_grid : (g_gcl_grid < 0 ? cdiv(nhalf, 2LL * -g_gcl_grid) : (conc > 1 ? std::max(1, device_cus() / 2) : device_cus()));
+                if (msum) {
+                    LAUNCH_LDS(F_GCL_EDGE, (k_gcl_edge_p<D, S1, S3, false, true>), std::min(nhalf, want), 8 * 64, (GclStream<D, 2>::LDS_BYTES / 2 * 3), st,
+                               tp, stream, P, Q, u0, c0, r0, r1, ew_in, ew_out, mbuf, GclTape{});
+                    return OARD_OK;
+                }
                 LAUNCH_LDS(F_GCL_EDGE, (k_gcl_edge_p<D, S1, S3>), std::min(nhalf, want), 8 * 64, (GclStream<D, 2>::LDS_BYTES / 2 * 3), st,
                            tp, stream, P, Q, u0, c0, r0, r1, ew_in, ew_out, mbuf, GclTape{});
+                return OARD_OK;
+            }
+            if (msum) {
+                LAUNCH_LDS(F_GCL_EDGE, (k_gcl_edge_v1<D, 8, 2, S1, S3, false, true, 2, 3>), cdiv(r1 - r0, 16 * 8), 8 * 64,
+                           (GclStream<D, 2>::LDS_BYTES / 2 * 3), st, tp, stream, P, Q, u0, c0, r0, r1, ew_in, ew_out, mbuf, GclTape{});
                 return OARD_OK;
             }
             GCL_RING3(false, GclTape{});
@@ -408,11 +427,11 @@
                        (GclRing<D, 2, 3>::LDS_BYTES), st, tp, stream, P, Q, u0, c0, r0, r1, ew_in, ew_out, mbuf, GclTape{}); return OARD_OK; }
         GCL_CASE(8, 8, 3)
         GCL_CASE(9, 8, 4)
-        case 10: { LAUNCH_LDS(F_GCL_EDGE, (k_gcl_edge_v1<D, 12, 1, S1, S3, false, 3>), cdiv(r1 - r0, 16 * 12), 12 * 64,
+        case 10: { LAUNCH_LDS(F_GCL_EDGE, (k_gcl_edge_v1<D, 12, 1, S1, S3, false, false, 3>), cdiv(r1 - r0, 16 * 12), 12 * 64,
                               (GclStream<D, 1>::LDS_BYTES), st, tp, stream, P, Q, u0, c0, r0, r1, ew_in, ew_out, mbuf, GclTape{}); return OARD_OK; }
-        case 11: { LAUNCH_LDS(F_GCL_EDGE, (k_gcl_edge_v1<D, 12, 2, S1, S3, false, 3>), cdiv(r1 - r0, 16 * 12), 12 * 64,
+        case 11: { LAUNCH_LDS(F_GCL_EDGE, (k_gcl_edge_v1<D, 12, 2, S1, S3, false, false, 3>), cdiv(r1 - r0, 16 * 12), 12 * 64,
                               (GclStream<D, 2>::LDS_BYTES), st, tp, stream, P, Q, u0, c0, r0, r1, ew_in, ew_out, mbuf, GclTape{}); return OARD_OK; }
-        case 12: { LAUNCH_LDS(F_GCL_EDGE, (k_gcl_edge_v1<D, 4, 1, S1, S3, false, 3>), cdiv(r1 - r0, 16 * 4), 4 * 64,
+        case 12: { LAUNCH_LDS(F_GCL_EDGE, (k_gcl_edge_v1<D, 4, 1, S1, S3, false, false, 3>), cdiv(r1 - r0, 16 * 4), 4 * 64,
                               (GclStream<D, 1>::LDS_BYTES), st, tp, stream, P, Q, u0, c0, r0, r1, ew_in, ew_out, mbuf, GclTape{}); return OARD_OK; }
 #endif
         default: return OARD_EINVAL;
@@ -420,10 +439,21 @@
 }
 template <class D>
 int launch_gcl_v1(int prec, int variant, int conc, const TopoDev& tp, const float* wb, const LayerOff& lo, const float* stream, const float* P, const float* Q, const float* u0,
-                  const float* c0, bool first, bool last, const float* ew_in, float* ew_out, float* mbuf, const GclTape* tape, hipStream_t st) {
+                  const float* c0, bool first, bool last, const float* ew_in, float* ew_out, float* mbuf, const GclTape* tape, hipStream_t st,
+                  bool msum = false) {
     const long long A = tp.A, E = tp.E;
     int rc;
     const bool skip = g_gcl_skip || tape;
+    if (msum) {
+        const long long c_in = tp.CI, c_all = tp.CI + tp.CX;
+        const bool s1 = !(skip && first), s3 = !(skip && last);
+        if (s1 && s3) return launch_gcl_v1s<D, true, true>(prec, variant, conc, tp, wb, lo, stream, P, Q, u0, c0, 0, c_all, ew_in, ew_out, mbuf, tape, st, true);
+        rc = launch_gcl_v1s<D, true, true>(prec, variant, conc, tp, wb, lo, stream, P, Q, u0, c0, 0, c_in, ew_in, ew_out, mbuf, tape, st, true);
+        if (rc != OARD_OK) return rc;
+        if (s1) return launch_gcl_v1s<D, true, false>(prec, variant, conc, tp, wb, lo, stream, P, Q, u0, c0, c_in, c_all, ew_in, ew_out, mbuf, tape, st, true);
+        if (s3) return launch_gcl_v1s<D, false, true>(prec, variant, conc, tp, wb, lo, stream, P, Q, u0, c0, c_in, c_all, ew_in, ew_out, mbuf, tape, st, true);
+        return launch_gcl_v1s<D, false, false>(prec, variant, conc, tp, wb, lo, stream, P, Q, u0, c0, c_in, c_all, ew_in, ew_out, mbuf, tape, st, true);
+    }
     if (!skip || (!first && !last)) return launch_gcl_v1s<D, true, true>(prec, variant, conc, tp, wb, lo, stream, P, Q, u0, c0, 0, E, ew_in, ew_out, mbuf, tape, st);
     rc = launch_gcl_v1s<D, true, true>(prec, variant, conc, tp, wb, lo, stream, P, Q, u0, c0, 0, A, ew_in, ew_out, mbuf, tape, st);
     if (rc != OARD_OK) return rc;
@@ -584,6 +614,10 @@
     float* vec2 = (float*)(ws + w.vec2);
     float* vcur = vec;
     float* vnext = vec2;
+    const bool msum = !train && g_gcl_msum && E > 0 && gcl_variant == 2 && node_variant == 1 && equi_variant != 0 && tp.npb > 4 &&
+                      (tp.CI == 0 || gcl_v1_throughput(c->precision, gcl_variant, topo->conc, tp.CI)) &&
+                      (tp.CX == 0 || gcl_v1_throughput(c->precision, gcl_variant, topo->conc, tp.CX));
+    g_gcl_msum_taken = msum;
     for (int l = 0; l < c->num_layers; ++l) {
         const LayerOff lo = po.layer[l];
         const bool nv1 = node_variant == 1 && equi_variant != 0;
@@ -603,13 +637,15 @@
                 GclTape gt{};
                 if (train) gt = GclTape{(float*)(tape + to.z1[l]), (float*)(tape + to.z2[l]), (float*)(tape + to.att[l]), (float*)(tape + to.z3[l])};
                 int rc = launch_gcl_v1<D>(c->precision, gcl_variant, topo->conc, tp, wb, lo, wb + lo.gcl_stream, P, Q, wb + po.u0, wb + po.c0row, l == 0,
-                                          l == c->num_layers - 1, ew_in, ew_out, mbuf, train ? &gt : nullptr, st);
+                                          l == c->num_layers - 1, ew_in, ew_out, mbuf, train ? &gt : nullptr, st, msum);
                 if (rc != OARD_OK) return rc;
             }
         }
         const bool rows = tp.npb <= 4;
         if (nv1 && rows) LAUNCH(F_NODE, (k_gcl_node_v1<D, NW, true>), gN16, NW * 64, st, tp, wb, lo, (const float*)xhb, (const float*)mbuf, s_mid_at(l), xq,
                                 train ? (float*)(tape + to.agg[l]) : nullptr);
+        else if (nv1 && msum) LAUNCH(F_NODE, (k_gcl_node_v1<D, NW, false, true>), gN16, NW * 64, st, tp, wb, lo, (const float*)xhb, (const float*)mbuf, s_mid_at(l), xq,
+                                     (float*)nullptr);
         else if (nv1) LAUNCH(F_NODE, (k_gcl_node_v1<D, NW, false>), gN16, NW * 64, st, tp, wb, lo, (const float*)xhb, (const float*)mbuf, s_mid_at(l), xq,
                              train ? (float*)(tape + to.agg[l]) : nullptr);
         else if constexpr (kV0) LAUNCH(F_NODE, (k_gcl_node<D>), gN, 256, st, tp, wb, lo, (const float*)xhb, (const float*)mbuf, s, xq);
@@ -1180,6 +1216,40 @@
     }
     std::vector<long long> ref_edge_ptr(N);
     for (int n = 0; n < N; ++n) ref_edge_ptr[n] = ref_ptr_ref[node_ref[n]];
+    std::vector<int> col_row, col_info, node_cols((size_t)N * 4, 0);
+    long long CI = 0, CX = 0;
+    {
+        auto pad16 = [&]() { while (col_row.size() % 16) col_row.push_back((int)E); };
+        for (int b = 0; b < B; ++b) {
+            for (int n = sample_ptr[b]; n < sample_ptr[b + 1]; ++n) {
+                const int q = node_sample[n] * n_obj + node_obj[n];
+                const int g0 = grp_ptr[q], g1 = grp_ptr[q + 1];
+                node_cols[4 * (size_t)n + 0] = (int)col_row.size();
+                for (int m = g0; m < g1; ++m) if (m != n) col_row.push_back(act_ptr[m] + (n - g0) - (n > m ? 1 : 0));
+                node_cols[4 * (size_t)n + 1] = (int)col_row.size();
+            }
+            pad16();
+        }
+        CI = (long long)col_row.size();
+        for (int b = 0; b < B; ++b) {
+            const int ns = sample_ptr[b + 1] - sample_ptr[b];
+            for (int n = sample_ptr[b]; n < sample_ptr[b + 1]; ++n) {
+                node_cols[4 * (size_t)n + 2] = (int)col_row.size();
+                for (long long e = edge_ptr[n]; e < (long long)edge_ptr[n] + ns - 1; ++e) if (edge_row[e] >= A) col_row.push_back(edge_row[e]);
+                node_cols[4 * (size_t)n + 3] = (int)col_row.size();
+            }
+            pad16();
+        }
+        CX = (long long)col_row.size() - CI;
+        if (CI + CX > 0x7fffffffLL - 256) return OARD_EINVAL;
+        if (col_row.empty()) col_row.push_back((int)E);
+        col_info.resize(col_row.size() * 4);
+        for (size_t k = 0; k < col_row.size(); ++k) {
+            const int r = col_row[k];
+            col_info[4 * k] = r; col_info[4 * k + 1] = row_src[r]; col_info[4 * k + 2] = row_tgt[r];
+            col_info[4 * k + 3] = r == (int)E ? -1 : row_src[r] + 1;
+        }
+    }
 
     std::vector<UploadItem> items;
     size_t cur = 0;
@@ -1192,7 +1262,8 @@
                  o_asrc = add(act_src.data(), act_src.size() * 4), o_atgt = add(act_tgt.data(), act_tgt.size() * 4),
                  o_aedge = add(act_edge.data(), act_edge.size() * 4), o_rptr = add(ref_edge_ptr.data(), N * 8),
                  o_erow = add(edge_row.data(), edge_row.size() * 4), o_rsrc = add(row_src.data(), row_src.size() * 4),
-                 o_rtgt = add(row_tgt.data(), row_tgt.size() * 4), o_reid = add(row_eid.data(), row_eid.size() * 4);
+                 o_rtgt = add(row_tgt.data(), row_tgt.size() * 4), o_reid = add(row_eid.data(), row_eid.size() * 4),
+                 o_crow = add(col_info.data(), col_info.size() * 4), o_ncol = add(node_cols.data(), node_cols.size() * 4);
     size_t cap = 0;
     char* dev = (char*)pool_alloc(cur, &cap);
     if (!dev) return OARD_EHIP;
@@ -1209,6 +1280,7 @@
     d.ref_edge_ptr = (const long long*)(dev + o_rptr);
     d.edge_row = (const int*)(dev + o_erow); d.row_src = (const int*)(dev + o_rsrc); d.row_tgt = (const int*)(dev + o_rtgt);
     d.row_eid = (const int*)(dev + o_reid);
+    d.CI = CI; d.CX = CX; d.col_info = (const int*)(dev + o_crow); d.node_cols = (const int*)(dev + o_ncol);
     return OARD_OK;
 }
 
@@ -2166,6 +2238,8 @@
     if (strcmp(name, "gcl_skip") == 0) { g_gcl_skip = value; return OARD_OK; }
     if (strcmp(name, "equi_skip") == 0) { g_equi_skip = value; return OARD_OK; }
     if (strcmp(name, "equi_l0_skip") == 0) { g_equi_l0_skip = value; return OARD_OK; }
+    if (strcmp(name, "gcl_msum") == 0) { g_gcl_msum = value; return OARD_OK; }
+    if (strcmp(name, "gcl_msum_taken") == 0) return g_gcl_msum_taken ? OARD_OK : OARD_EINVAL;
     if (strcmp(name, "equi_l0_taken") == 0) return g_equi_l0_taken ? OARD_OK : OARD_EINVAL;
     if (strcmp(name, "gcl_persist") == 0) { g_gcl_persist = value; return OARD_OK; }
     if (strcmp(name, "gcl_grid") == 0) { g_gcl_grid = value; return OARD_OK; }
diff --git a/oareactdiff_amd/csrc/oard_inst.h b/oareactdiff_amd/csrc/oard_inst.h
--- a/oareactdiff_amd/csrc/oard_inst.h
+++ b/oareactdiff_amd/csrc/oard_inst.h
@@ -16,7 +16,8 @@
 #define OARD_A_GCL (TopoDev, const float*, const float*, const float*, const float*, const float*, long long, long long, const float*, float*, float*, GclTape)
 
 #if !defined(OARD_INST_DEFINE) || defined(OARD_INST_UNIT_GCL_P)
-#define OARD_I_GCL_P(D, S1, S3) OARD_INST((k_gcl_edge_p<OARD_UNPAREN D, S1, S3, false>), OARD_A_GCL) OARD_INST((k_gcl_edge_p<OARD_UNPAREN D, S1, S3, true>), OARD_A_GCL)
+#define OARD_I_GCL_P(D, S1, S3) OARD_INST((k_gcl_edge_p<OARD_UNPAREN D, S1, S3, false>), OARD_A_GCL) OARD_INST((k_gcl_edge_p<OARD_UNPAREN D, S1, S3, true>), OARD_A_GCL) \
+    OARD_INST((k_gcl_edge_p<OARD_UNPAREN D, S1, S3, false, true>), OARD_A_GCL)
 #define X(h, r) OARD_BOOL4(OARD_I_GCL_P, (Dims<h, r>))
 OARD_DIMS_LIST
 #undef X
@@ -24,8 +25,9 @@
 
 #if !defined(OARD_INST_DEFINE) || defined(OARD_INST_UNIT_GCL_V1)
 #define OARD_I_GCL_V1(D, S1, S3) \
-    OARD_INST((k_gcl_edge_v1<OARD_UNPAREN D, 8, 2, S1, S3, false, 2, 3>), OARD_A_GCL) OARD_INST((k_gcl_edge_v1<OARD_UNPAREN D, 8, 2, S1, S3, true, 2, 3>), OARD_A_GCL) \
-    OARD_INST((k_gcl_edge_v1<OARD_UNPAREN D, 4, 2, S1, S3, false, 2, 2>), OARD_A_GCL) \
+    OARD_INST((k_gcl_edge_v1<OARD_UNPAREN D, 8, 2, S1, S3, false, false, 2, 3>), OARD_A_GCL) OARD_INST((k_gcl_edge_v1<OARD_UNPAREN D, 8, 2, S1, S3, true, false, 2, 3>), OARD_A_GCL) \
+    OARD_INST((k_gcl_edge_v1<OARD_UNPAREN D, 8, 2, S1, S3, false, true, 2, 3>), OARD_A_GCL) \
+    OARD_INST((k_gcl_edge_v1<OARD_UNPAREN D, 4, 2, S1, S3, false, false, 2, 2>), OARD_A_GCL) \
     OARD_INST((k_gcl_edge_small<OARD_UNPAREN D, 8, S1, S3>), (TopoDev, const float*, LayerOff, const float*, const float*, const float*, const float*, long long, long long, float*, float*))
 #define X(h, r) OARD_BOOL4(OARD_I_GCL_V1, (Dims<h, r>))
 OARD_DIMS_LIST
@@ -63,6 +65,7 @@
 #define OARD_A_MSG_BWD (TopoDev, const float*, Strided3, Strided3, const float*, Strided3, const float*, int, Strided3, float*, float*, float*, float*, int, int, int)
 #define X(h, r) \
     OARD_INST((k_gcl_node_v1<Dims<h, r>, OARD_NW(h), false>), OARD_A_GCL_NODE) OARD_INST((k_gcl_node_v1<Dims<h, r>, OARD_NW(h), true>), OARD_A_GCL_NODE) \
+    OARD_INST((k_gcl_node_v1<Dims<h, r>, OARD_NW(h), false, true>), OARD_A_GCL_NODE) \
     OARD_INST((k_out_v1<Dims<h, r>, OARD_NW(h)>), OARD_A_OUT) \
     OARD_INST((k_scalarize_bwd<Dims<h, r>, 2, false>), OARD_A_SCAL_BWD) OARD_INST((k_scalarize_bwd<Dims<h, r>, 2, true>), OARD_A_SCAL_BWD) \
     OARD_INST((k_equi_msg_bwd<Dims<h, r> >), OARD_A_MSG_BWD)
diff --git a/oareactdiff_amd/csrc/oard_layout.h b/oareactdiff_amd/csrc/oard_layout.h
--- a/oareactdiff_amd/csrc/oard_layout.h
+++ b/oareactdiff_amd/csrc/oard_layout.h
@@ -68,6 +68,9 @@
     const int *grp_ptr;
     const int *act_ptr, *act_src, *act_tgt, *act_edge;
     const long long *ref_edge_ptr;
+    long long CI, CX;
+    const int *col_info;
+    const int *node_cols;
 };
 
 struct ActList {
diff --git a/oareactdiff_amd/csrc/oard_node_v1.h b/oareactdiff_amd/csrc/oard_node_v1.h
--- a/oareactdiff_amd/csrc/oard_node_v1.h
+++ b/oareactdiff_amd/csrc/oard_node_v1.h
@@ -287,11 +287,12 @@
     }
 }
 
-template <class D, int WAVES, bool ROWS = false>
+template <class D, int WAVES, bool ROWS = false, bool MSUM = false>
 __global__ __launch_bounds__(WAVES * 64) void k_gcl_node_v1(TopoDev tp, const float* __restrict__ wb, LayerOff lo,
                                                             const float* __restrict__ xh, const float* __restrict__ mbuf,
                                                             float* __restrict__ s, float* __restrict__ xq,
                                                             float* __restrict__ agg_out ) {
+    static_assert(!(MSUM && ROWS), "the partial sums exist for the large-batch gather only");
     __shared__ __attribute__((aligned(16))) float sm[4 * D::HT * 256];
     float* in = sm;
     float* hm = sm + 2 * D::HT * 256;
@@ -302,6 +303,19 @@
     const size_t e0 = (size_t)tp.edge_ptr[nb.n];
     const int mx = wave_max(deg);
     const float inv = 1.0f / (float)max(deg, 1);
+    int in_lo = 0, x_lo = 0, n_in = 0, cnt = 0;
+    if (MSUM) {
+        const int* nc = tp.node_cols + 4 * (size_t)nb.n;
+        const int in_hi = nc[1], x_hi = nc[3];
+        in_lo = nc[0]; x_lo = nc[2];
+        n_in = (nb.valid && in_hi > in_lo) ? 1 + ((in_hi - 1) >> 4) - (in_lo >> 4) : 0;
+        cnt = n_in + ((nb.valid && x_hi > x_lo) ? 1 + ((x_hi - 1) >> 4) - (x_lo >> 4) : 0);
+    }
+    auto pc = [&](int k) -> size_t {
+        const int lo = k < n_in ? in_lo : x_lo, j = k < n_in ? k : k - n_in;
+        return (size_t)(j == 0 ? lo : ((lo >> 4) + j) << 4);
+    };
+    const int mxp = MSUM ? wave_max(cnt) : 0;
     for (int t = nb.wave; t < D::HT; t += WAVES) {
         lds_st(in, t, nb.lane, ld_blk(xh, nb.n, D::HP, t, nb.lane));
         f4 a0 = f4zero(), a1 = f4zero();
@@ -322,7 +336,17 @@
             a1 = f4zero();
         }
         const int last = max(deg - 1, 0);
-        for (int k = 0; !ROWS && k < mx; k += 8) {
+        for (int k = 0; MSUM && k < mxp; k += 8) {
+            f4 r[8];
+#pragma unroll
+            for (int i = 0; i < 8; ++i) r[i] = ld_blk(mbuf, pc(min(k + i, max(cnt - 1, 0))), D::HP, t, nb.lane);
+#pragma unroll
+            for (int i = 0; i < 8; ++i) {
+                const f4 v = k + i < cnt ? r[i] : f4zero();
+                if (i & 1) a1 += v; else a0 += v;
+            }
+        }
+        for (int k = 0; !ROWS && !MSUM && k < mx; k += 8) {
             f4 r[8];
 #pragma unroll
             for (int i = 0; i < 8; ++i) r[i] = ld_blk(mbuf, e0 + min(k + i, last), D::HP, t, nb.lane);
```
